# JuanTarrio/rebvo

Measured on AMD Instinct MI355X. Metric: frames/sec (DoG+extract+track+depth) 752x480 EuRoC, higher is better.
Workload: dtype f32 scale-space / f64 tracker+EKF

## Files before the change

### include/edgehip.h

```cpp
#ifndef EDGEHIP_H
#define EDGEHIP_H
#include <stdint.h>

#ifdef __cplusplus
extern "C" {
#endif

#define EDGEHIP_ABI_VERSION 2
#define EDGEHIP_KEYLINE_MAX 50000

typedef enum edgehip_status {
    EDGEHIP_OK = 0,
    EDGEHIP_ERR_ARG = -1,
    EDGEHIP_ERR_DEVICE = -2,
    EDGEHIP_ERR_MEMORY = -3,
    EDGEHIP_ERR_STATE = -4
} edgehip_status;

typedef struct edgehip_ctx edgehip_ctx;

typedef struct edgehip_params {
    int32_t w, h;
    double ppx, ppy, zfx, zfy;
    double kc[5];
// ... 28 lines not shown
    int32_t p_id, n_id, net_id, stereo_m_id;
    double stereo_rho, stereo_s_rho;
} edgehip_keyline;

typedef struct edgehip_seq_state {
    double tresh;
    double V[3], W[3];
    double P_V[9], P_W[9];
    double R[9];
    double Pose[9], Pos[3];
    double Kp, P_Kp, K;
    double s_rho_q;
    double score, rel_error, rel_error_score;
    double t_prev, dt;
    float retuned_thresh;
    int32_t l_kl_num;
    int32_t frame;
    int32_t klm_fwd;
    int32_t klm_num, kf_matchs;
    int32_t estimation_ok;
    int32_t minimizer_evals;
} edgehip_seq_state;

typedef struct edgehip_nav {
    double t, dt;
    double V[3], W[3], P_V[9], P_W[9];
    double Rot[9], RotLie[3], Vel[3], Pose[9], PoseLie[3], Pos[3];
    double Kp, RKp, s_rho_q, tresh, score, rel_error, rel_error_score;
    float retuned_thresh;
    int32_t kn, klm_fwd, klm_num, kf_matchs, estimation_ok, frame, minimizer_evals;
} edgehip_nav;

typedef struct edgehip_imu_params {
    double giro_meas_std, giro_bias_std;
    int32_t init_bias, init_bias_frame_num;
    double bias_init_guess[3];
    double acel_meas_std, g_module, g_module_uncer, g_uncert, vbias_std;
    double scale_std_mult, scale_std_max, scale_std_init;
} edgehip_imu_params;
typedef struct edgehip_imu_integrated {
    int32_t n, pad;
    double dt, Rot[9], giro[3], acel[3], comp[3], dgiro[3], cacel[3];
} edgehip_imu_integrated;
typedef struct edgehip_nav_imu {
    double Rot[9], RotLie[3], RotGiro[3], Vel[3], Pose[9], PoseLie[3], Pos[3], g[3];
    double scale, dt, K, Kp, RKp, s_rho_q;
    double Vg[3], Bg[3], dVv[3], dWv[3], Vgv[3], Vgva[3], Av[3], As[3], X[7], b_est[3], u_est[3];
    int32_t kn, klm_num, estimation_ok, init;
} edgehip_nav_imu;

int edgehip_create(const edgehip_params *params, int nseq, int nslots, int device, edgehip_ctx **out);
int edgehip_destroy(edgehip_ctx *ctx);
const char *edgehip_last_error(void);
int edgehip_abi_version(void);
int edgehip_experiments(void);
int edgehip_sync(edgehip_ctx *ctx);
void *edgehip_stream(edgehip_ctx *ctx);
int edgehip_box_widths(edgehip_ctx *ctx, int out[6]);

int edgehip_upload_rgb(edgehip_ctx *ctx, int slot, const uint8_t *rgb24, int seq_first, int count);
int edgehip_upload_rgb_device(edgehip_ctx *ctx, int slot, const void *rgb24_dev);
int edgehip_alloc_pinned(size_t bytes, void **out);
int edgehip_free_pinned(void *p);
int edgehip_upload_rgb_pinned(edgehip_ctx *ctx, int slot, const uint8_t *rgb24_pinned, int seq_first, int count);
int edgehip_upload_sync(edgehip_ctx *ctx);
int edgehip_upload_wait(edgehip_ctx *ctx, int slot);

int edgehip_upload_rgb_indexed(edgehip_ctx *ctx, int slot, const void *pool_dev, int pool_frames, const int32_t *idx);
int edgehip_bind_rgb_indexed(edgehip_ctx *ctx, int slot, const void *pool_dev, int pool_frames, const int32_t *idx);
int edgehip_upload_grey8(edgehip_ctx *ctx, int slot, const uint8_t *grey8, int seq_first, int count);
int edgehip_upload_grey8_pinned(edgehip_ctx *ctx, int slot, const uint8_t *grey8_pinned, int seq_first, int count);
int edgehip_bind_grey8_indexed(edgehip_ctx *ctx, int slot, const void *pool_dev, int pool_frames, const int32_t *idx);

int edgehip_stage_a(edgehip_ctx *ctx, int slot);
int edgehip_get_kn(edgehip_ctx *ctx, int slot, int32_t *kn_out);

int edgehip_quantile(edgehip_ctx *ctx, int slot, double s_rho_min, double s_rho_max, double pct, int nbins);
int edgehip_build_field(edgehip_ctx *ctx, int slot, int radius, float min_mod);
int edgehip_try_velrot(edgehip_ctx *ctx, int slot_new, int slot_old, const double *X, int reweight, int procjf,
                       double match_thresh, const double *s_rho_min, uint32_t match_num_thresh, double k_huber,
                       int resid_in, int resid_out, double *out);
int edgehip_download_resid(edgehip_ctx *ctx, int which, double *resid);
int edgehip_minimizer_rv(edgehip_ctx *ctx, int slot_new, int slot_old);
int edgehip_set_tracker_precision(edgehip_ctx *ctx, int bits);
int edgehip_lm_solve(edgehip_ctx *ctx, const double *A, const double *b, int n, int svd_rule, double *h);

typedef struct edgehip_kf_request {
    double X0[6];
    double Kr;
    double max_s_rho;
} edgehip_kf_request;
typedef struct edgehip_kf_result {
    double X[6];
    double RRV[36];
    double score_ratio;
    double F, F0;
    int32_t evals, mnum;
} edgehip_kf_result;
int edgehip_minimizer_rv_kf(edgehip_ctx *ctx, int slot_kf, int slot_cur, const edgehip_kf_request *req, double match_mod,
                            double match_ang, double rho_tol, int iter_max, double reweight_distance, uint32_t match_num_thresh,
                            edgehip_kf_result *res);

int edgehip_minimizer_v(edgehip_ctx *ctx, int slot_new, int slot_old, double *V, const double *s_rho_min, float min_mod,
                        double match_thresh, int iter_max, uint32_t match_num_thresh, double reweight_distance,
                        double *RVel, double *F);

int edgehip_forward_match(edgehip_ctx *ctx, int slot_old, int slot_new);
int edgehip_rotate_keylines(edgehip_ctx *ctx, int slot, const double *R );
int edgehip_directed_matching(edgehip_ctx *ctx, int slot_new, int slot_old);
int edgehip_match_one_pass(edgehip_ctx *ctx, int slot_new, int slot_old, int fill);
int edgehip_regularize_ekf(edgehip_ctx *ctx, int slot, int do_regularize, int do_ekf);
int edgehip_ext_rot_vel(edgehip_ctx *ctx, int slot, const double *vel, double loc_unc, double hub_reweight, double *X,
                        double *Wx, double *Rx, int32_t *ok);
int edgehip_rescale(edgehip_ctx *ctx, int slot);

int edgehip_set_slot_camera(edgehip_ctx *ctx, int slot, double ppx, double ppy, double zfx, double zfy);
int edgehip_directed_matching_stereo(edgehip_ctx *ctx, int slot, int slot_pair, const double *t, const double *R,
                                     double min_thr_mod, double min_thr_ang, double max_radius, double loc_unc,
                                     double q_abs, double q_rel, double loc_unc_model, int32_t *nmatch);
int edgehip_fuse_stereo_depth(edgehip_ctx *ctx, int slot);
int edgehip_set_stereo_rig(edgehip_ctx *ctx, int slot_pair, const double *t, const double *R, double max_radius);
int edgehip_get_stereo_matches(edgehip_ctx *ctx, int32_t *nmatch);

int edgehip_process_frame(edgehip_ctx *ctx, const double *t);
int edgehip_next_slot(edgehip_ctx *ctx);
int edgehip_cur_slot(edgehip_ctx *ctx);
int edgehip_read_nav(edgehip_ctx *ctx, edgehip_nav *nav);
int edgehip_imu_enable(edgehip_ctx *ctx, const edgehip_imu_params *imu);
int edgehip_set_imu(edgehip_ctx *ctx, const edgehip_imu_integrated *per_seq);
int edgehip_read_nav_imu(edgehip_ctx *ctx, edgehip_nav_imu *out);
int edgehip_set_nav_log(edgehip_ctx *ctx, int len);
int edgehip_read_nav_log(edgehip_ctx *ctx, int first, int count, edgehip_nav *out);
int edgehip_read_nav_log_device(edgehip_ctx *ctx, int first, int count, void *out_dev);
int edgehip_read_nav_imu_log(edgehip_ctx *ctx, int first, int count, edgehip_nav_imu *out);
int edgehip_read_stereo_matches_log(edgehip_ctx *ctx, int first, int count, int32_t *out);
int edgehip_reset(edgehip_ctx *ctx);
int edgehip_depth_reset(edgehip_ctx *ctx, int seq);
int edgehip_depth_reset_slot(edgehip_ctx *ctx, int seq, int slot);

int edgehip_get_state(edgehip_ctx *ctx, int seq, edgehip_seq_state *out);
int edgehip_set_state(edgehip_ctx *ctx, int seq, const edgehip_seq_state *in);
int edgehip_get_framecount(edgehip_ctx *ctx, int seq, int slot, uint32_t *fc);
int edgehip_set_framecount(edgehip_ctx *ctx, int seq, int slot, uint32_t fc);
int edgehip_download_keylines(edgehip_ctx *ctx, int seq, int slot, edgehip_keyline *kl, int32_t *mask,
                              int32_t *kn_out);
int edgehip_download_keylines_batch(edgehip_ctx *ctx, int slot, int n, const int32_t *seqs, edgehip_keyline *const *kl, int32_t *kn_out);
int edgehip_export_keylines(edgehip_ctx *ctx, int n, const int32_t *seqs, int *ticket_out);
int edgehip_export_fetch(edgehip_ctx *ctx, int ticket, const int32_t *kn, edgehip_keyline *const *dst);
int edgehip_export_wait(edgehip_ctx *ctx, int ticket);
int edgehip_register_host(void *p, size_t bytes);
int edgehip_unregister_host(void *p);
int edgehip_upload_keylines(edgehip_ctx *ctx, int seq, int slot, const edgehip_keyline *kl, int32_t kn,
                            const int32_t *mask, float retuned_thresh);
int edgehip_download_plane(edgehip_ctx *ctx, int seq, int which, float *out);
int edgehip_download_field(edgehip_ctx *ctx, int seq, int32_t *out);
int edgehip_build_undistort_map(const edgehip_params *params, int32_t *inx, int32_t *iw);
int edgehip_download_undistorted(edgehip_ctx *ctx, int seq, int slot, uint8_t *rgb24);

typedef enum edgehip_bound_mode {
    EDGEHIP_BOUND_NONE = 0,
    EDGEHIP_BOUND_CORNERS = 1,
    EDGEHIP_BOUND_FULL = 2
} edgehip_bound_mode;
typedef struct edgehip_depth_fill_params {
    int32_t block_w, block_h;
    int32_t iter_num;
// ... 192 lines not shown
```

### rebvo_amd/csrc/api.hip

```cpp

#include <math.h>
#include <stdio.h>
#include <stdlib.h>
#include <string.h>

#include <algorithm>
#include <mutex>

#include "ctx.h"
#include "stage_a_dev.h"

namespace edgehip {

static thread_local std::string g_err;

int wait_pinned_ring(edgehip_ctx *c) {
    const int r = c->frames_seen % 8;
    if (c->ring_valid[r]) EH_CHECK(hipEventSynchronize(c->ev_ring[r]));
    return 0;
}

static int wait_idx_row(edgehip_ctx *c, int slot, const int32_t *pi) {
    if (c->slot_src[slot].idx_row != pi) return 0;
    if (c->a_api_valid[slot]) EH_CHECK(hipEventSynchronize(c->ev_a[slot]));
// ... 354 lines not shown
        EH_CHECK(hipEventCreateWithFlags(&c->ev_a[i], hipEventDisableTiming));
        EH_CHECK(hipEventCreateWithFlags(&c->ev_use[i], hipEventDisableTiming));
        c->use_valid[i] = false;
    }
    EH_CHECK(hipEventCreateWithFlags(&c->ev_tmp, hipEventDisableTiming));
    EH_CHECK(hipEventCreateWithFlags(&c->ev_stage, hipEventDisableTiming));
    EH_CHECK(hipEventCreateWithFlags(&c->ev_stage8, hipEventDisableTiming));
    for (int i = 0; i < 8; i++) { EH_CHECK(hipEventCreateWithFlags(&c->ev_ring[i], hipEventDisableTiming)); c->ring_valid[i] = false; }
    if (nslots > 4) { set_error("edgehip_create: at most 4 frame slots"); return EDGEHIP_ERR_ARG; }

    DevicePlan &pl = c->plan;
    pl.w = p.w; pl.h = p.h; pl.n = p.w * p.h; pl.nseq = nseq; pl.nslots = nslots;
    pl.ftx = (p.w + 3) / 4;
    pl.fstride = (size_t)pl.ftx * (size_t)((p.h + 3) / 4) * 16;
    pl.f16tx = (p.w + 7) / 8;
    pl.f16stride = (size_t)pl.f16tx * (size_t)((p.h + 3) / 4) * 32;
    pl.cap = std::min(p.max_points, EDGEHIP_KEYLINE_MAX);
    const double sr0 = kovesi_boxes(p.sigma0, kMaxBoxes, pl.box[0]);
    kovesi_boxes(sr0 * p.ksigma, kMaxBoxes, pl.box[1]);
    for (int f = 0; f < 2; f++)
        for (int i = 0; i < kMaxBoxes; i++) {
            if (pl.box[f][i] < 1 || pl.box[f][i] * pl.box[f][i] >= kDivLutMax) {
                set_error("edgehip_create: box width out of range for these sigmas");
                return EDGEHIP_ERR_ARG;
            }
            pl.box_a[f][i] = (float)(1.0 / (pl.box[f][i] * pl.box[f][i]));
        }
    pl.ppx = (float)p.ppx; pl.ppy = (float)p.ppy; pl.zfx = (float)p.zfx; pl.zfy = (float)p.zfy;
    pl.zfm = (double)((pl.zfx + pl.zfy) / 2);

    const size_t B = nseq, S = nslots, N = pl.n, CAP = pl.cap;
    int e;
#define EH_TRY(x) if ((e = (x)) != 0) return e
    EH_TRY(dmalloc(c, &c->rgb, S * B * N * 3 + 16, al->dev, 0));
    EH_TRY(dmalloc(c, &c->ii, 4 * B * N, al->dev, 0));
    c->planes = nullptr;
    if (p.debug_planes) EH_TRY(dmalloc(c, &c->planes, 5 * B * N, al->dev, 0));
    EH_TRY(dmalloc(c, &c->mask, S * B * N, al->dev, 0xFF));
    EH_TRY(dmalloc(c, &c->field, B * pl.fstride, al->dev, 0xFF));
    EH_TRY(dmalloc(c, &c->field16, B * pl.f16stride, al->dev, 0));
    c->field32_valid = false;
    c->und_base = nullptr;
    c->und_iw = nullptr;
    if (p.use_undistort) {
        EH_TRY(dmalloc(c, &c->und_base, N, al->dev));
        EH_TRY(dmalloc(c, &c->und_iw, N, al->dev));
        std::vector<int32_t> base;
        std::vector<uint32_t> iw;
        build_undistort_map(p, base, iw, nullptr, nullptr);
        EH_CHECK(hipMemcpy(c->und_base, base.data(), sizeof(int32_t) * N, hipMemcpyHostToDevice));
        EH_CHECK(hipMemcpy(c->und_iw, iw.data(), sizeof(uint32_t) * 4 * N, hipMemcpyHostToDevice));
    }
    EH_TRY(dmalloc(c, &c->div_lut, kDivLutMax, al->dev));
    EH_TRY(dmalloc(c, &c->pinv, 3 * 49, al->dev, 0));
    EH_TRY(dmalloc(c, &c->seq, B, al->dev, 0));
    EH_TRY(dmalloc(c, &c->seqa, B, al->dev, 0));
    EH_TRY(dmalloc(c, &c->tresh_slot, S * B, al->dev, 0));
    c->fc_rows = std::max<int>(nslots, kRefRing);
    c->fc_index = 0;
    EH_TRY(dmalloc(c, &c->framecount, (size_t)c->fc_rows * B, al->dev, 0));
    EH_TRY(dmalloc(c, &c->kn_slot, S * B, al->dev, 0));
    EH_TRY(dmalloc(c, &c->retuned_slot, S * B, al->dev, 0));
    c->band_rows = detect_band_rows(p.w, p.plane_fit_size);
    c->nbands = (p.h - 2 * p.plane_fit_size + c->band_rows - 1) / c->band_rows;
    {
        const int npx = c->band_rows * p.w, nchunk = (npx + 63) / 64, cpw = (nchunk + kDetWaves - 1) / kDetWaves;
        c->band_cap = cpw * 64;
    }
    const size_t nstrips = (size_t)c->nbands * kDetWaves;
    EH_TRY(dmalloc(c, &c->band_cnt, B * nstrips, al->dev, 0));
    EH_TRY(dmalloc(c, &c->band_off, B * (nstrips + 1), al->dev, 0));
    {
        char *bs;
        EH_TRY(dmalloc(c, &bs, B * nstrips * c->band_cap * 20, al->dev));
        c->band_stage = bs;
    }
    EH_TRY(dmalloc(c, &c->histo, B * 256, al->dev, 0));
    c->nblk_tvr = (int)((CAP + kTvrBlock - 1) / kTvrBlock);
    EH_TRY(dmalloc(c, &c->P0, B * 3 * CAP, al->dev, 0));
    EH_TRY(dmalloc(c, &c->resid, (size_t)kResidBufs * B * CAP, al->dev, 0));
    EH_TRY(dmalloc(c, &c->resid_carry, (size_t)kResidBufs * B * c->nblk_tvr, al->dev, 0));
    EH_TRY(dmalloc(c, &c->partials, 2 * B * c->nblk_tvr * kNumSums, al->dev, 0));
    EH_TRY(dmalloc(c, &c->block_last, 2 * B * c->nblk_tvr, al->dev, 0));
    EH_TRY(dmalloc(c, &c->bin_cnt, B * 256, al->dev, 0));
    {
        const size_t ntiles = (size_t)((p.w + 63) / 64) * ((p.h + 63) / 64);
        EH_TRY(dmalloc(c, &c->bins, B * ntiles * CAP, al->dev));
    }
    c->field_radius = p.search_range;
    c->field_mode = EH_EXP_ENV("EDGEHIP_FIELD_MODE", 0);
    c->no_grec = getenv("EDGEHIP_NO_GREC") && atoi(getenv("EDGEHIP_NO_GREC")) != 0;
    c->level_mode = getenv("EDGEHIP_LEVEL_MODE") ? atoi(getenv("EDGEHIP_LEVEL_MODE")) : 0;
    c->fwd_mode = EH_EXP_ENV("EDGEHIP_FWD_MODE", 0);
    c->fused_min_batch = fused_min_env;
    c->fused_undist = EH_EXP_ENV("EDGEHIP_FUSED_UNDIST", 0) != 0;
    c->tvr_rw2 = EH_EXP_ENV("EDGEHIP_TVR_RW2", 0);
    c->dual_init = getenv("EDGEHIP_DUAL_INIT") ? atoi(getenv("EDGEHIP_DUAL_INIT")) : 1;
    c->persist_lm_max = EH_EXP_ENV("EDGEHIP_PERSIST_LM", 0);
    EH_TRY(dmalloc(c, &c->sync_cnt, B, al->dev, 0));
    EH_TRY(dmalloc(c, &c->fwd_key, B * CAP, al->dev, 0));
    EH_TRY(dmalloc(c, &c->fwd_win, B * CAP, al->dev, 0xFF));
    EH_TRY(dmalloc(c, &c->rs_tmp, B * 2 * CAP, al->dev, 0));
    c->fuse_match = !(getenv("EDGEHIP_FUSE_MATCH") && atoi(getenv("EDGEHIP_FUSE_MATCH")) == 0);
    if (c->fuse_match) {
        EH_TRY(dmalloc(c, &c->rot_pm, S * B * CAP, al->dev, 0)); EH_TRY(dmalloc(c, &c->rot_mm, S * B * CAP, al->dev, 0));
        EH_TRY(dmalloc(c, &c->rot_rho, S * B * CAP, al->dev, 0)); EH_TRY(dmalloc(c, &c->rot_srho, S * B * CAP, al->dev, 0));
    }
    EH_TRY(dmalloc(c, &c->rot_buf, B * 9, al->dev, 0));
    EH_TRY(dmalloc(c, &c->nav_dev, B, al->dev, 0));
    EH_TRY(dmalloc(c, &c->idx_dev, B, al->dev, 0));
    c->slot_src.assign(S, edgehip_ctx::SlotSrc());
    c->stereo_cnt = nullptr;
    if (p.stereo_available) EH_TRY(dmalloc(c, &c->stereo_cnt, B, al->dev, 0));
    c->nav_log = nullptr;
    c->nav_log_len = 0;

    {
        const size_t al256 = 256;
        auto up = [&](size_t x) { return (x + al256 - 1) / al256 * al256; };
        const bool stereo = p.stereo_available != 0;
        const size_t per = up(CAP * 4) * 8  +
                           up(CAP * 8) * 6  + up(CAP * 8) * 7  + up(CAP * 32) + up(CAP * 16)  +
                           (stereo ? up(CAP * 4) + 2 * up(CAP * 8) : 0);
        char *arena;
        EH_TRY(dmalloc(c, &arena, per * S * B, al->dev, 0));
        c->kl_arena = arena;
        c->kl.resize(S * B);
        for (size_t sb = 0; sb < S * B; sb++) {
            char *q = arena + sb * per;
            KlSoA &k = c->kl[sb];
            auto take = [&](size_t bytes) { char *r = q; q += up(bytes); return r; };
            k.p_inx = (int32_t *)take(CAP * 4);
            k.m_m = (float2 *)take(CAP * 8); k.u_m = (float2 *)take(CAP * 8); k.c_p = (float2 *)take(CAP * 8);
            k.p_m = (float2 *)take(CAP * 8); k.p_m_0 = (float2 *)take(CAP * 8); k.m_m0 = (float2 *)take(CAP * 8);
            k.n_m = (float *)take(CAP * 4);
            k.rho = (double *)take(CAP * 8); k.s_rho = (double *)take(CAP * 8); k.rho_nr = (double *)take(CAP * 8);
            k.s_rho_nr = (double *)take(CAP * 8); k.rho0 = (double *)take(CAP * 8); k.s_rho0 = (double *)take(CAP * 8);
            k.n_m0 = (double *)take(CAP * 8);
            k.m_id = (int32_t *)take(CAP * 4); k.m_id_f = (int32_t *)take(CAP * 4); k.m_id_kf = (int32_t *)take(CAP * 4);
            k.m_num = (int32_t *)take(CAP * 4); k.p_id = (int32_t *)take(CAP * 4); k.n_id = (int32_t *)take(CAP * 4);
            k.rec = (MatchRec *)take(CAP * 32);
            k.grec = (float4 *)take(CAP * 16);
            k.stereo_m_id = nullptr; k.stereo_rho = nullptr; k.stereo_s_rho = nullptr;
            if (stereo) {
                k.stereo_m_id = (int32_t *)take(CAP * 4);
                k.stereo_rho = (double *)take(CAP * 8); k.stereo_s_rho = (double *)take(CAP * 8);
            }
        }
        c->slot_cam.assign(S, edgehip_ctx::SlotCam{pl.ppx, pl.ppy, pl.zfm});
        EH_TRY(dmalloc(c, &c->kl_dev, S * B, al->dev));
        EH_CHECK(hipMemcpyAsync(c->kl_dev, c->kl.data(), sizeof(KlSoA) * S * B, hipMemcpyHostToDevice, c->stream));
    }
    {
        std::vector<float> lut(kDivLutMax, 0.f);
        for (int k = 1; k < kDivLutMax; k++) lut[k] = (float)(1.0 / (double)(float)k);
        EH_CHECK(hipMemcpyAsync(c->div_lut, lut.data(), sizeof(float) * kDivLutMax, hipMemcpyHostToDevice, c->stream));
        double pinv[3 * 49] = {0};
        plane_fit_pinv(p.plane_fit_size, pinv);
        if (p.plane_fit_size == 2)
            for (int i = 0; i < 5; i++)
                for (int j = 0; j < 5; j++) {
                    const int k = i * 5 + j;
                    if (!(pinv[k] == pinv[j] && pinv[25 + k] == pinv[25 + 5 * i] && pinv[50 + k] == pinv[50])) {
                        set_error("edgehip_create: plane-fit pseudo inverse lost its separable structure");
                        return EDGEHIP_ERR_STATE;
                    }
// ... 999 lines not shown
```

### rebvo_amd/csrc/ctx.h

```cpp
#pragma once
#include <hip/hip_runtime.h>
#include <stdint.h>
#include <string.h>
#include <string>
#include <map>
#include <vector>
#include <mutex>
#include <atomic>

#include "edgehip.h"
#include "export_ring.h"

namespace edgehip {

constexpr int kMaxBoxes = 3;
constexpr int kBandRows = 12;
constexpr int kDetWaves = 16;
constexpr int kDivLutMax = 256;
constexpr int kTvrThreads = 256;
constexpr int kTvrBlock = kTvrThreads;
constexpr int kNumSums = 28;
constexpr int kRefRing = 8;
constexpr int kResidBufs = 3;

// ... 266 lines not shown
    typedef T __attribute__((address_space(1))) G;
    __builtin_nontemporal_store(v, (G *)p + i);
#else
    st_stream(p + i, v);
#endif
}
__device__ __forceinline__ void stg_stream(float2 *p, size_t i, float2 v) {
#if EDGEHIP_GLOBAL_LD
    typedef float f2v __attribute__((ext_vector_type(2)));
    typedef f2v __attribute__((address_space(1))) G;
    __builtin_nontemporal_store(f2v{v.x, v.y}, (G *)p + i);
#else
    st_stream(p + i, v);
#endif
}
#endif

struct Profiler;

}

struct edgehip_ctx {
    edgehip_params p;
    edgehip::DevicePlan plan;
    int device;
    hipStream_t stream;
    hipStream_t stream_a;
    hipEvent_t ev_a[4];
    hipEvent_t ev_use[4];
    hipEvent_t ev_tmp;
    hipEvent_t ev_stage, ev_stage8;
    bool stage_busy = false, stage8_busy = false;
    hipStream_t stream_up;
    hipEvent_t ev_up[4];
    bool up_valid[4];
    int slot_ring[4];
    bool no_grec;
    bool grec_ok[4];
    bool rec_stale[4];
    bool rig_a_valid = false;
    bool capturing = false;
    bool a_api_valid[4];
    hipEvent_t ev_ring[8];
    bool ring_valid[8];
    bool use_valid[4];
    int overlap;
    bool lds_optin_level = false, lds_optin_detect = false, lds_optin_fused = false;
    bool lds_optin_rescale = false;
    int frame_slot;
    int frames_seen;
    uint8_t *rgb;
    float *ii;
    float *planes;
    int32_t *mask;
    uint32_t *field;
    uint16_t *field16;
    bool field32_valid;
    int32_t *und_base;
    uint4 *und_iw;
    float *div_lut;
    double *pinv;
    void *kl_arena;
    std::vector<edgehip::KlSoA> kl;
    edgehip::KlSoA *kl_dev;
    edgehip::SeqDev *seq;
    edgehip::SeqA *seqa;
    double *tresh_slot;
    uint32_t *framecount;
    int fc_rows;
    int fc_index;
    int32_t *kn_slot;
    float *retuned_slot;
    int32_t *band_cnt;
    int32_t *band_off;
    void *band_stage;
    int nbands, band_cap;
    int band_rows;
    int32_t *histo;
    double *P0;
    double *resid;
    double *resid_carry;
    double *partials;
    double *block_last;
    bool use_graph;
    std::map<int, hipGraphExec_t> frame_graphs;
    struct StereoRig {
        bool enabled = false;
        int slot_pair = -1;
        double t[3], R[9], max_radius;
    } rig;
    int ring_slots;
    struct SlotSrc { const uint8_t *base = nullptr; std::vector<int32_t> host_idx; bool grey8 = false;
                     const int32_t *idx_row = nullptr; int idx_ring = 0; };
    uint8_t *grey8 = nullptr;
    uint8_t *pinned_grey8 = nullptr;
    std::vector<SlotSrc> slot_src;
    struct SlotCam { float ppx, ppy; double zfm; };
    std::vector<SlotCam> slot_cam;
    int field_radius;
    int field_mode;
    int level_mode;
    int fused_min_batch;
    double pinv_host[3 * 49];
    int32_t *bin_cnt;
    int32_t *bins;
    int nblk_tvr;
    bool fused_undist;
    int tvr_rw2;
    bool tracker_f32 = false;
    int dual_init;
    int persist_lm_max;
    unsigned *sync_cnt;
    unsigned long long *fwd_key;
    int32_t *fwd_win;
    int fwd_mode = 0;
    bool fuse_match = true;
    float2 *rot_pm = nullptr, *rot_mm = nullptr;
    double *rot_rho = nullptr, *rot_srho = nullptr;
    bool rot_pending[4] = {false, false, false, false};
    bool fwd_fill[4] = {false, false, false, false};
    bool fwd_cleared = false;
    bool fwd_keys_posted = false;
    bool fwd_key_in_tvr = false;
    double *rs_tmp;
    double *rot_buf;
    const double *t_src = nullptr;
    edgehip_keyline *aos_dev = nullptr;
    edgehip_keyline *aos_host = nullptr;
    int32_t *aos_req_dev = nullptr, *aos_req_host = nullptr;
    int aos_requests = 0;
    edgehip::ExportRing kl_ring;
    edgehip::ExportRing ros_ring;
    edgehip_nav *nav_dev;
    edgehip_nav *nav_log;
    edgehip_nav_imu *nav_imu_log = nullptr;
    int nav_log_len;
    int32_t *stereo_log = nullptr;
    hipStream_t stream_log = nullptr;
    hipEvent_t ev_log = nullptr;
    hipEvent_t ev_log_ring[8] = {};
    std::mutex log_mu;
    std::atomic<long long> frames_logged{0};
    long long log_first = 0, log_last = -1;
    int32_t *idx_dev;
    int32_t *stereo_cnt;
    uint8_t *pinned_rgb;
    size_t pinned_rgb_bytes;
    edgehip::SeqDev *pinned_seq;
    edgehip::SeqA *pinned_seqa;
    double *pinned_out;
    double *pinned_t;
    int32_t *pinned_idx;
    edgehip_nav *pinned_nav;
    edgehip::Profiler *prof;
    bool imu_enabled = false, imu_pending = false;
    bool imu_pinned_ok = false;
    edgehip_imu_params imu_params;
    edgehip_kf_request *kf_req_dev = nullptr;
    edgehip_kf_result *kf_res_dev = nullptr;
    void *imu_track = nullptr;
    void *imu_filter = nullptr;
    void *imu_snap = nullptr;
    hipStream_t stream_imu = nullptr;
    hipEvent_t ev_imu_snap[2], ev_imu_post[2];
    hipEvent_t ev_imu_mid[2];
    bool imu_post_valid[2] = {false, false};
// ... 168 lines not shown
```

### rebvo_amd/csrc/stage_b.hip

```cpp

#include <math.h>
#include <string.h>

#include <vector>

#include <type_traits>

#include "ctx.h"
#include "resid_carry.h"
#include "wave_reduce.h"

namespace edgehip {

struct RetuneArgs {
    SeqA *seqa;
    const int32_t *histo;
    float *retuned_out;
    int knum, nbins;
};
template <int NT>
__global__ __launch_bounds__(NT) void k_quantile(const KlSoA *kls, const int32_t *__restrict__ kns, SeqDev *seqs,
                                                 double smin, double smax, double pct, int nbins, const double *__restrict__ t_in, double fps,
                                                 RetuneArgs rt) {
    __shared__ int s_h[256];
// ... 403 lines not shown
                acc_abl += val | off;
#else
                atomicMin(px, val);
#endif
            };
            constexpr int UNROLL = EDGEHIP_RASTER_UNROLL;
            const float t1f = (float)t1;
            float tf = (float)t0;
            if constexpr (UNROLL > 1) {
                for (; tf + (float)(UNROLL - 1) <= t1f; tf += (float)UNROLL) {
#pragma unroll
                    for (int j = 0; j < UNROLL; j++) sample(tf + (float)j);
                }
            }
            for (; tf <= t1f; tf += 1.f) sample(tf);
#if EDGEHIP_RASTER_ABL == 2
            if (acc_abl == 0x12345u) s_tile[1] = acc_abl;
#endif
        }
    };
    using T = std::true_type;
    using F = std::false_type;
    if (tx0 == 0) { if (ty0 == 0) raster(T{}, T{}); else raster(T{}, F{}); }
    else { if (ty0 == 0) raster(F{}, T{}); else raster(F{}, F{}); }
    __syncthreads();
    if (tid == 0) bin_cnt[(size_t)seq * kMaxTiles + tile] = 0;
#if EDGEHIP_RASTER_ABL == 4
    if (s_tile[tid] != 0x12345u) return;
#endif
    if (keep32) {
        uint32_t *out = field + (size_t)seq * fstride;
        for (int i = tid; i < FT * FT; i += 256) {
            const int st = i >> 4, in = i & 15;
            const int lx = ((st % (FT / 4)) << 2) | (in & 3), ly = ((st / (FT / 4)) << 2) | (in >> 2);
            const int x = tx0 + lx, y = ty0 + ly;
            if (x < w && y < h) out[field_index(x, y, ftx)] = s_tile[ly * TS + lx];
        }
    }
    uint16_t *o16 = field16 + (size_t)seq * f16stride;
    for (int i = tid; i < FT * FT / 2; i += 256) {
        const int st = i >> 4, in = i & 15;
        const int lx = ((st % (FT / 8)) << 3) | ((in & 3) << 1), ly = ((st / (FT / 8)) << 2) | (in >> 2);
        const int x = tx0 + lx, y = ty0 + ly;
        if (x < w && y < h) {
            const uint32_t v0 = s_tile[ly * TS + lx], v1 = s_tile[ly * TS + lx + 1];
            const uint32_t a0 = v0 == 0xFFFFFFFFu ? 0u : ((0x10000u - (v0 & 0xFFFFu)) & 0xFFFFu);
            const uint32_t a1 = v1 == 0xFFFFFFFFu ? 0u : ((0x10000u - (v1 & 0xFFFFu)) & 0xFFFFu);
#if EDGEHIP_NT_RASTER
            st_stream(reinterpret_cast<uint32_t *>(o16 + field16_index(x, y, f16tx)), a0 | (a1 << 16));
#else
            *reinterpret_cast<uint32_t *>(o16 + field16_index(x, y, f16tx)) = a0 | (a1 << 16);
#endif
        }
    }
}

__global__ __launch_bounds__(256) void k_field_to16(const uint32_t *__restrict__ field, uint16_t *__restrict__ f16, int w, int h,
                                                    size_t fstride, int ftx, size_t f16stride, int f16tx) {
    const int seq = blockIdx.z;
    const size_t e = (size_t)blockIdx.x * 256 + threadIdx.x;
    if (e >= f16stride) return;
    const size_t tile = e >> 5; const int in = (int)(e & 31);
    const int x = (int)(tile % (size_t)f16tx) * 8 + (in & 7), y = (int)(tile / (size_t)f16tx) * 4 + (in >> 3);
    uint16_t v = 0;
    if (x < w && y < h) {
        const uint32_t f = field[(size_t)seq * fstride + field_index(x, y, ftx)];
        if (f != 0xFFFFFFFFu) v = (uint16_t)(0xFFFF - (int)(f & 0xFFFFu) + 1);
    }
    f16[(size_t)seq * f16stride + e] = v;
}

__global__ __launch_bounds__(256) void k_tvr_prepare(const KlSoA *kls, const int32_t *__restrict__ kns, double *__restrict__ P0,
                                                     double *__restrict__ resid0, double *__restrict__ carry0, SeqDev *seqs,
                                                     int cap, int nblk, double zfm) {
    const int seq = blockIdx.z;
    const int i = blockIdx.x * 256 + threadIdx.x;
    const int kn = kns[seq];
    if (i == 0) seqs[seq].kn_old = kn;
    if ((i % kTvrBlock) == 0 && i / kTvrBlock < nblk) carry0[(size_t)seq * nblk + i / kTvrBlock] = 0.0;
    if (i >= kn) return;
    resid0[(size_t)seq * cap + i] = 0.0;
}

__device__ __forceinline__ void so3_exp_inl(const double (&w)[3], double (&R)[9]) {
    const double one_6th = 1.0 / 6.0, one_20th = 1.0 / 20.0;
    const double theta_sq = w[0] * w[0] + w[1] * w[1] + w[2] * w[2];
    const double theta = sqrt(theta_sq);
    double A, B;
    if (theta_sq < 1e-8) {
        A = 1.0 - one_6th * theta_sq;
        B = 0.5;
    } else if (theta_sq < 1e-6) {
        B = 0.5 - 0.25 * one_6th * theta_sq;
        A = 1.0 - theta_sq * one_6th * (1.0 - one_20th * theta_sq);
    } else {
        const double inv_theta = 1.0 / theta;
        A = sin(theta) * inv_theta;
        B = (1 - cos(theta)) * (inv_theta * inv_theta);
    }
    const double wx2 = w[0] * w[0], wy2 = w[1] * w[1], wz2 = w[2] * w[2];
    R[0] = 1.0 - B * (wy2 + wz2);
    R[4] = 1.0 - B * (wx2 + wz2);
    R[8] = 1.0 - B * (wx2 + wy2);
    double a = A * w[2], b = B * (w[0] * w[1]);
    R[1] = b - a; R[3] = b + a;
    a = A * w[1]; b = B * (w[0] * w[2]);
    R[2] = b + a; R[6] = b - a;
    a = A * w[0]; b = B * (w[1] * w[2]);
    R[5] = b - a; R[7] = b + a;
}
__device__ __noinline__ void so3_exp(const double w[3], double R[9]) {
    const double wv[3] = {w[0], w[1], w[2]};
    double Rr[9];
    so3_exp_inl(wv, Rr);
    for (int i = 0; i < 9; i++) R[i] = Rr[i];
}

__device__ __noinline__ void tvr_setup(SeqDev *sq, const double *X) {
    double R0[9], Rz[9];
    so3_exp(X + 3, R0);
    const double wz[3] = {0.0, 0.0, X[5]};
    so3_exp(wz, Rz);
    for (int i = 0; i < 9; i++) sq->Rt[i] = R0[i];
    sq->RM[0] = Rz[0]; sq->RM[1] = Rz[1]; sq->RM[2] = Rz[3]; sq->RM[3] = Rz[4];
    for (int i = 0; i < 3; i++) sq->Vt[i] = X[i];
}


__device__ __forceinline__ void tvr_setup2(SeqDev *sq, const double *X, const int lane, const bool zero = false, const int l0 = 0) {
    if (lane >= l0 && lane < l0 + 2) {
        const bool first = lane == l0;
        const double wv[3] = {first ? X[3] : 0.0, first ? X[4] : 0.0, X[5]};
        double R[9];
        so3_exp_inl(wv, R);
        double *Rt = zero ? sq->zRt : sq->Rt, *Vt = zero ? sq->zVt : sq->Vt, *RM = zero ? sq->zRM : sq->RM;
        if (first) {
            for (int i = 0; i < 9; i++) Rt[i] = R[i];
            for (int i = 0; i < 3; i++) Vt[i] = X[i];
        } else {
            RM[0] = R[0]; RM[1] = R[1]; RM[2] = R[3]; RM[3] = R[4];
        }
    }
}


struct TvrArgs {
    const KlSoA *kl_old;
    const KlSoA *kl_new;
    const int32_t *kn_old;
    const uint16_t *field16;
    const double *P0;
    double *resid;
    double *resid_carry;
    double *block_last;
    double *partials;
    double *block_last_z;
    double *partials_z;
    SeqDev *seq;
    const uint32_t *framecount;
    int w, h, cap, nblk, nseq;
    size_t f16stride;
    int f16tx;
    double zfm, max_r, match_thresh, k_huber, inv_k_huber;
    double inv_zfm;
    float ppx, ppy;
    uint32_t match_num_thresh;
    int write_mid;
    int use_grec;
    unsigned long long *fwd_key;
    const edgehip_kf_request *kf;
    double kf_match_mod, kf_match_cang, kf_rho_tol;
};

__device__ __forceinline__ double rsqrt_f64(double x) {
    double y = __builtin_amdgcn_rsq(x);
    const double hx = 0.5 * x;
    y = y * (1.5 - hx * y * y);
    y = y * (1.5 - hx * y * y);
    return x > 1e300 ? 0.0 : y;
}

#ifndef EDGEHIP_TVR_MFMA
#define EDGEHIP_TVR_MFMA 0
#endif
#ifndef EDGEHIP_TVR_REF_ORDER
#define EDGEHIP_TVR_REF_ORDER 1
#endif
#ifndef EDGEHIP_TVR_ABL
#define EDGEHIP_TVR_ABL 0
#endif
template <bool GREC>
__device__ __forceinline__ void load_matched(const KlSoA &kl, const int ikf, float &cpx, float &cpy, float &mx, float &my, float &ux, float &uy) {
    if (GREC) {
        const float4 g = ldg(kl.grec, ikf);
        cpx = g.x; cpy = g.y; mx = g.z; my = g.w;
    } else {
        const MatchRec fr = kl.rec[ikf];
        cpx = fr.c_px; cpy = fr.c_py; mx = fr.m_mx; my = fr.m_my; ux = fr.u_mx; uy = fr.u_my;
    }
}
__device__ __forceinline__ void grec_u_m(const float mx, const float my, float &ux, float &uy) {
    const float n2m = mx * mx + my * my;
    const float nm = sqrtf_mid(n2m);
    div2_mid_f32(mx, my, nm, ux, uy);
}

template <typename T>
__device__ __forceinline__ void jac_row(T (&J)[6], const T zf, const T rho_p, const T pix, const T piy, const T ptx, const T pty, const T ptz,
                                        const T dfx, const T dfy) {
    T t0 = zf * rho_p;
    J[0] = t0 * dfx;
    J[1] = t0 * dfy;
    t0 = rho_p * pix;
    J[2] = t0 * dfx;
    t0 = rho_p * piy;
    J[2] += t0 * dfy;
    J[3] = J[1] * ptz; J[3] += J[2] * pty;
    J[4] = J[0] * ptz; J[4] += J[2] * ptx;
    t0 = J[0] * pty;
    J[5] = (T)-1 * t0; J[5] += J[1] * ptx;
}

template <bool REWEIGHT, bool PROCJF, bool GREC, bool KF = false>
__device__ __forceinline__ void tvr_body(const TvrArgs &a, const int seq, const int blk, const int tid) {
    constexpr int ABL = KF ? 0 : EDGEHIP_TVR_ABL;
    const int lane = tid & 63, wave = tid >> 6;
    SeqDev *sq = a.seq + seq;
    const int kn = a.kn_old[seq];
    if (blk * kTvrBlock >= kn) return;
    const KlSoA &ko = a.kl_old[seq];
    const int res_in = sq->res_cur, res_out = sq->lm_phase == 0 ? sq->res_t : sq->res_new;
    const double *rin = a.resid + ((size_t)res_in * a.nseq + seq) * a.cap;
    double *rout = a.resid + ((size_t)res_out * a.nseq + seq) * a.cap;
    const double carry_in_prev = a.resid_carry[((size_t)res_in * a.nseq + seq) * a.nblk + blk];

    constexpr int NW = kTvrThreads / 64;
    constexpr bool GRAM_MFMA = PROCJF && EDGEHIP_TVR_MFMA && !(ABL & 1);
    __shared__ double s_rows[GRAM_MFMA ? NW : 1][GRAM_MFMA ? 64 : 1][8];
    __shared__ double s_wlast[NW];
    __shared__ int s_whas[NW];
    double sums[kNumSums];
#pragma unroll
    for (int i = 0; i < kNumSums; i++) sums[i] = 0;

    const int ikl = blk * kTvrBlock + tid;
    double J[6] = {0, 0, 0, 0, 0, 0};
    double fm, dfx, dfy;
    double ptx, pty, ptz, pix, piy, rho_p, s_rho;
#if EDGEHIP_TVR_REF_ORDER
    double wgt_ref;
#else
    double inv_w2 = 1;
#endif
    int mid_f = -1;
    int status = 0;
    double fi = 0;
    double rho_own;
    if (ikl < kn) {
        s_rho = ldg(ko.s_rho, ikl);
        const int32_t mnum = ldg(ko.m_num, ikl);
        const float2 pm0 = ldg(ko.p_m, ikl);
        const double rho0 = ldg(ko.rho, ikl);
        rho_own = rho0;
        const float2 klm = ldg(ko.m_m, ikl);
        const float knm = ldg(ko.n_m, ikl);
        double rprev = 0;
        if (REWEIGHT && !(ABL & 16)) rprev = rin[ikl];
        const uint32_t fc = KF ? 0xFFFFFFFFu : a.framecount[seq];
        const uint32_t mthr = a.match_num_thresh < fc ? a.match_num_thresh : fc;
        const bool skip = s_rho > sq->s_rho_min_eval || (uint32_t)mnum < mthr;
        if (!skip) {
            const double sz = inv_mid(rho0);
            const double pz_zf0 = a.inv_zfm * sz;
            const double sx = pz_zf0 * (double)pm0.x, sy = pz_zf0 * (double)pm0.y;
            const double *R = sq->Rt, *V = sq->Vt;
            ptx = R[0] * sx; ptx += R[1] * sy; ptx += R[2] * sz; ptx = V[0] + ptx;
            pty = R[3] * sx; pty += R[4] * sy; pty += R[5] * sz; pty = V[1] + pty;
            ptz = R[6] * sx; ptz += R[7] * sy; ptz += R[8] * sz; ptz = V[2] + ptz;
            rho_p = inv_mid(ptz);
            const double pz_zf = a.zfm * rho_p;
            pix = pz_zf * ptx;
            piy = pz_zf * pty;
            const double px = pix + (double)a.ppx, py = piy + (double)a.ppy;
            const int x = cvt_trunc_sat_i32(px + 0.5), y = cvt_trunc_sat_i32(py + 0.5);
            dfx = 0; dfy = 0;
#if EDGEHIP_TVR_REF_ORDER
            wgt_ref = 1;
#endif
            if (REWEIGHT) {
                if (is_carry(rprev)) rprev = carry_in_prev;
#if EDGEHIP_TVR_REF_ORDER
                if (fabs(rprev) > a.k_huber) wgt_ref = div_mid(a.k_huber, fabs(rprev));
#else
                if (fabs(rprev) > a.k_huber && !(ABL & 2)) { const double rk = fabs(rprev) * a.inv_k_huber; inv_w2 = rk * rk; }
#endif
            }
            fm = a.max_r;
            if (x < 1 || y < 1 || x >= a.w - 1 || y >= a.h - 1) {
                status = 1;
            } else {
                status = 3;
                const float rmx = KF ? klm.x : (float)(sq->RM[0] * (double)klm.x + sq->RM[1] * (double)klm.y);
                const float rmy = KF ? klm.y : (float)(sq->RM[2] * (double)klm.x + sq->RM[3] * (double)klm.y);
                const uint32_t f = (ABL & 8) ? (uint32_t)(ikl + 1) : a.field16[(size_t)seq * a.f16stride + field16_index(x, y, a.f16tx)];
                if (KF) {
                    if (f != 0u) {
                        const int ikf = (int)f - 1;
                        const KlSoA &kf = a.kl_new[seq];
                        const MatchRec fr = kf.rec[ikf];
                        const double f_rho = kf.rho[ikf], f_srho = kf.s_rho[ikf];
                        const double cang = (double)((klm.x * fr.m_mx + klm.y * fr.m_my) / knm);
                        const double rho_t = rho_p / a.kf[seq].Kr;
                        const bool reject = cang < a.kf_match_cang || (double)fabsf(knm / fr.n_m - 1) > a.kf_match_mod ||
                                            fabs(rho_t - f_rho) > a.kf_rho_tol * (f_srho + s_rho * rho_t / rho0);
                        if (!reject) {
                            const double dx = px - (double)fr.c_px, dy = py - (double)fr.c_py;
                            fi = dx * (double)fr.u_mx + dy * (double)fr.u_my;
                            dfx = (double)fr.u_mx;
                            dfy = (double)fr.u_my;
                            fm = fi;
                            mid_f = ikf;
                            status = 2;
                        }
                    }
                } else {
                    const int ikf = f != 0u ? (int)f - 1 : 0;
                    float f_cpx, f_cpy, f_mx, f_my, f_ux, f_uy;
                    if (ABL & 4) {
                        f_cpx = (float)px; f_cpy = (float)py; f_mx = klm.x; f_my = klm.y; f_ux = 1.f; f_uy = 0.f;
                    } else {
                        load_matched<GREC>(a.kl_new[seq], ikf, f_cpx, f_cpy, f_mx, f_my, f_ux, f_uy);
                    }
                    const double p_n2 = (double)(knm * knm);
                    const double p_esc = (double)(rmx * f_mx + rmy * f_my);
                    if ((f != 0u) & !(fabs(p_esc - p_n2) > a.match_thresh * p_n2)) {
                        if (GREC) grec_u_m(f_mx, f_my, f_ux, f_uy);
                        const double dx = px - (double)f_cpx, dy = py - (double)f_cpy;
                        fi = dx * (double)f_ux + dy * (double)f_uy;
                        dfx = (double)f_ux;
                        dfy = (double)f_uy;
                        fm = fi;
                        mid_f = ikf;
                        status = 2;
                    }
                }
            }
        }
    }

    {
        const WaveLast<double> wl = wave_last_valid(fi, status == 2, lane);
        carry_publish(wl, lane, wave, s_wlast, s_whas);
        __syncthreads();
        if (status == 3) {
            rout[ikl] = carry_inherit(wl, wave, s_wlast, s_whas);
        } else if (status == 2) {
            rout[ikl] = fi;
        } else if (status == 1) {
            rout[ikl] = a.max_r;
        } else if (ikl < kn) {
            rout[ikl] = 0.0;
        }
    }
    if (a.write_mid && ikl < kn) {
        stg(ko.m_id_f, ikl, mid_f);
        if (!KF && a.fwd_key && mid_f >= 0) atomicMax(&a.fwd_key[(size_t)seq * a.cap + mid_f], ord_bits(rho_own));
    }

    double fs = 0;
    if (status != 0) {
#if EDGEHIP_TVR_REF_ORDER
        if (REWEIGHT) { fm *= wgt_ref; dfx *= wgt_ref; dfy *= wgt_ref; }
#endif
        if (PROCJF) jac_row(J, a.zfm, rho_p, pix, piy, ptx, pty, ptz, dfx, dfy);
        const double qvel = (a.zfm * dfx * sq->Vt[0] + a.zfm * dfy * sq->Vt[1] + (pix * dfx + piy * dfy) * sq->Vt[2]);
#if EDGEHIP_TVR_REF_ORDER
        const double q_rho = REWEIGHT ? sqrt_ge1(s_rho * qvel * s_rho * qvel + 1) : s_rho;
        const double r_q = rcp_for_div_rn(q_rho);
        if (PROCJF) {
#pragma unroll
            for (int j = 0; j < 6; j++) J[j] = div_rn(J[j], q_rho, r_q);
        }
        fs = div_rn(fm, q_rho, r_q);
#else
        double inv_q;
        if (REWEIGHT) {
            const double sq = s_rho * qvel;
            inv_q = (ABL & 2) ? sq + inv_w2 : rsqrt_f64(sq * sq + inv_w2);
        } else {
            inv_q = 1.0 / s_rho;
        }
        if (PROCJF) {
#pragma unroll
            for (int j = 0; j < 6; j++) J[j] *= inv_q;
        }
        fs = fm * inv_q;
#endif
    } else if (!REWEIGHT && !KF && ikl < kn && s_rho == 0) {
        const double qnan = __longlong_as_double(0x7ff8000000000000ll);
        if (PROCJF) {
#pragma unroll
            for (int j = 0; j < 6; j++) J[j] = qnan;
        }
        fs = qnan;
    }
    if (GRAM_MFMA) {
        double2 *row = reinterpret_cast<double2 *>(&s_rows[wave][lane][0]);
        row[0] = make_double2(J[0], J[1]);
        row[1] = make_double2(J[2], J[3]);
        row[2] = make_double2(J[4], J[5]);
        row[3] = make_double2(fs, 0.0);
    } else {
        int ns = 0;
        if (PROCJF) {
#pragma unroll
            for (int i = 0; i < 6; i++)
#pragma unroll
                for (int j = i; j < 6; j++) sums[ns++] = J[i] * J[j];
#pragma unroll
            for (int i = 0; i < 6; i++) sums[ns++] = J[i] * fs;
        }
        sums[PROCJF ? ns : kNumSums - 1] = fs * fs;
    }

    if (tid == 0) a.block_last[(size_t)seq * a.nblk + blk] = carry_block_last(s_wlast, s_whas);

    __shared__ double s_red[NW][32];
    if (GRAM_MFMA) {
        typedef double v4d __attribute__((ext_vector_type(4)));
        __builtin_amdgcn_fence(__ATOMIC_RELEASE, "wavefront");
        __builtin_amdgcn_wave_barrier();
        const int m = (lane & 15) < 7 ? (lane & 15) : 7, kk = lane >> 4;
        const double *src = &s_rows[wave][kk][m];
        v4d acc = {0.0, 0.0, 0.0, 0.0};
#pragma unroll
        for (int st = 0; st < 16; st++) {
            const double v = src[st * 4 * 8];
            acc = __builtin_amdgcn_mfma_f64_16x16x4f64(v, v, acc, 0, 0, 0);
        }
        const int j = lane & 15;
#pragma unroll
        for (int r = 0; r < 2; r++) {
            const int i = (lane >> 4) + 4 * r;
            if (j < 7 && i <= j) {
                const int idx = j < 6 ? i * 6 - (i * (i - 1)) / 2 + (j - i) : (i < 6 ? 21 + i : 27);
                s_red[wave][idx] = acc[r];
            }
        }
    } else if (PROCJF && (ABL & 1)) {
        if (lane < kNumSums) s_red[wave][lane] = sums[lane % 4];
    } else {
        block_reduce_put<PROCJF>(sums, lane, wave, s_red);
    }
    __syncthreads();
    block_reduce_store<PROCJF>(s_red, tid, a.partials + ((size_t)seq * a.nblk + blk) * kNumSums);
}

template <bool REWEIGHT, bool PROCJF, bool GREC>
__global__ __launch_bounds__(kTvrThreads) void k_try_velrot(TvrArgs a) {
    tvr_body<REWEIGHT, PROCJF, GREC>(a, blockIdx.z, blockIdx.x, threadIdx.x);
}
__global__ __launch_bounds__(kTvrThreads) void k_try_velrot_kf(TvrArgs a) {
    tvr_body<true, true, false, true>(a, blockIdx.z, blockIdx.x, threadIdx.x);
}

template <bool REWEIGHT, bool PROCJF, bool GREC>
__device__ __forceinline__ void tvr_body_f32(const TvrArgs &a, const int seq, const int blk, const int tid) {
    const int lane = tid & 63, wave = tid >> 6;
    SeqDev *sq = a.seq + seq;
    const int kn = a.kn_old[seq];
    if (blk * kTvrBlock >= kn) return;
    const KlSoA &ko = a.kl_old[seq];
    const int res_in = sq->res_cur, res_out = sq->lm_phase == 0 ? sq->res_t : sq->res_new;
    const double *rin = a.resid + ((size_t)res_in * a.nseq + seq) * a.cap;
    double *rout = a.resid + ((size_t)res_out * a.nseq + seq) * a.cap;
    const double carry_in_prev = a.resid_carry[((size_t)res_in * a.nseq + seq) * a.nblk + blk];
    constexpr int NW = kTvrThreads / 64;
    __shared__ float s_wlast[NW];
    __shared__ int s_whas[NW];
    float sums[kNumSums];
#pragma unroll
    for (int i = 0; i < kNumSums; i++) sums[i] = 0.f;

    const int ikl = blk * kTvrBlock + tid;
    float J[6] = {0, 0, 0, 0, 0, 0};
    float fm, dfx, dfy;
    float ptx, pty, ptz, pix, piy, rho_p;
    double s_rho;
    float wgt;
    int mid_f = -1, status = 0;
    float fi = 0;
    double rho_own;
    const float zf = (float)a.zfm, max_r = (float)a.max_r, k_huber = (float)a.k_huber, simil_t = (float)a.match_thresh;
    float Vt0, Vt1, Vt2;
    if (ikl < kn) {
        s_rho = ldg(ko.s_rho, ikl);
        const int32_t mnum = ldg(ko.m_num, ikl);
        const float2 pm0 = ldg(ko.p_m, ikl);
        const double rho0 = ldg(ko.rho, ikl);
        rho_own = rho0;
        const float2 klm = ldg(ko.m_m, ikl);
        const float knm = ldg(ko.n_m, ikl);
        double rprev_d = 0;
        if (REWEIGHT) rprev_d = rin[ikl];
        const uint32_t fc = a.framecount[seq];
        const uint32_t mthr = a.match_num_thresh < fc ? a.match_num_thresh : fc;
        const bool skip = s_rho > sq->s_rho_min_eval || (uint32_t)mnum < mthr;
        Vt0 = (float)sq->Vt[0]; Vt1 = (float)sq->Vt[1]; Vt2 = (float)sq->Vt[2];
        if (!skip) {
            const float sz = 1.f / (float)rho0;
            const float pz_zf0 = (1.f / zf) * sz;
            const float sx = pz_zf0 * pm0.x, sy = pz_zf0 * pm0.y;
            const double *Rd = sq->Rt;
            const float R0 = (float)Rd[0], R1 = (float)Rd[1], R2 = (float)Rd[2], R3 = (float)Rd[3], R4 = (float)Rd[4], R5 = (float)Rd[5],
                        R6 = (float)Rd[6], R7 = (float)Rd[7], R8 = (float)Rd[8];
            ptx = R0 * sx; ptx += R1 * sy; ptx += R2 * sz; ptx = Vt0 + ptx;
            pty = R3 * sx; pty += R4 * sy; pty += R5 * sz; pty = Vt1 + pty;
            ptz = R6 * sx; ptz += R7 * sy; ptz += R8 * sz; ptz = Vt2 + ptz;
            rho_p = 1.f / ptz;
            const float pz_zf = zf * rho_p;
            pix = pz_zf * ptx;
            piy = pz_zf * pty;
            const float px = pix + a.ppx, py = piy + a.ppy;
            const int x = cvt_trunc_sat_i32((double)px + 0.5), y = cvt_trunc_sat_i32((double)py + 0.5);
            dfx = 0; dfy = 0; wgt = 1;
            if (REWEIGHT) {
                if (is_carry(rprev_d)) rprev_d = carry_in_prev;
                const float rprev = (float)rprev_d;
                if (fabsf(rprev) > k_huber) wgt = k_huber / fabsf(rprev);
            }
            fm = max_r;
            if (x < 1 || y < 1 || x >= a.w - 1 || y >= a.h - 1) {
                status = 1;
            } else {
                status = 3;
                const float rmx = (float)sq->RM[0] * klm.x + (float)sq->RM[1] * klm.y;
                const float rmy = (float)sq->RM[2] * klm.x + (float)sq->RM[3] * klm.y;
                const uint32_t f = a.field16[(size_t)seq * a.f16stride + field16_index(x, y, a.f16tx)];
                {
                    const int ikf = f != 0u ? (int)f - 1 : 0;
                    float f_cpx, f_cpy, f_mx, f_my, f_ux, f_uy;
                    load_matched<GREC>(a.kl_new[seq], ikf, f_cpx, f_cpy, f_mx, f_my, f_ux, f_uy);
                    const float p_n2 = knm * knm;
                    const float p_esc = rmx * f_mx + rmy * f_my;
                    if ((f != 0u) & !(fabsf(p_esc - p_n2) > simil_t * p_n2)) {
                        if (GREC) grec_u_m(f_mx, f_my, f_ux, f_uy);
                        const float dx = px - f_cpx, dy = py - f_cpy;
                        fi = dx * f_ux + dy * f_uy;
                        dfx = f_ux;
                        dfy = f_uy;
                        fm = fi;
                        mid_f = ikf;
                        status = 2;
                    }
                }
            }
        }
    }
    {
        const WaveLast<float> wl = wave_last_valid(fi, status == 2, lane);
        carry_publish(wl, lane, wave, s_wlast, s_whas);
        __syncthreads();
        if (status == 3) {
            rout[ikl] = carry_inherit(wl, wave, s_wlast, s_whas);
        } else if (status == 2) {
            rout[ikl] = (double)fi;
        } else if (status == 1) {
            rout[ikl] = (double)max_r;
        } else if (ikl < kn) {
            rout[ikl] = 0.0;
        }
    }
    if (a.write_mid && ikl < kn) {
        stg(ko.m_id_f, ikl, mid_f);
        if (a.fwd_key && mid_f >= 0) atomicMax(&a.fwd_key[(size_t)seq * a.cap + mid_f], ord_bits(rho_own));
    }
    float fs = 0.f;
    if (status != 0) {
        if (REWEIGHT) { fm *= wgt; dfx *= wgt; dfy *= wgt; }
        if (PROCJF) jac_row(J, zf, rho_p, pix, piy, ptx, pty, ptz, dfx, dfy);
        const double qvel = (double)(zf * dfx * Vt0 + zf * dfy * Vt1 + (pix * dfx + piy * dfy) * Vt2);
        const double q_rho = REWEIGHT ? sqrt_ge1(s_rho * qvel * s_rho * qvel + 1) : s_rho;
        const double r_q = rcp_for_div_rn(q_rho);
        if (PROCJF) {
#pragma unroll
            for (int j = 0; j < 6; j++) J[j] = (float)div_rn((double)J[j], q_rho, r_q);
        }
        fs = (float)div_rn((double)fm, q_rho, r_q);
    }
    {
        int ns = 0;
        if (PROCJF) {
#pragma unroll
            for (int i = 0; i < 6; i++)
#pragma unroll
                for (int j = i; j < 6; j++) sums[ns++] = J[i] * J[j];
#pragma unroll
            for (int i = 0; i < 6; i++) sums[ns++] = J[i] * fs;
        }
        sums[PROCJF ? ns : kNumSums - 1] = fs * fs;
    }
    if (tid == 0) a.block_last[(size_t)seq * a.nblk + blk] = carry_block_last(s_wlast, s_whas);
    __shared__ float s_red[NW][32];
    block_reduce_put<PROCJF>(sums, lane, wave, s_red);
    __syncthreads();
    block_reduce_store<PROCJF>(s_red, tid, a.partials + ((size_t)seq * a.nblk + blk) * kNumSums);
}
template <bool REWEIGHT, bool PROCJF, bool GREC>
__global__ __launch_bounds__(kTvrThreads) void k_try_velrot_f32(TvrArgs a) {
    tvr_body_f32<REWEIGHT, PROCJF, GREC>(a, blockIdx.z, blockIdx.x, threadIdx.x);
}

#ifndef EDGEHIP_TVR2_PARK
#define EDGEHIP_TVR2_PARK 1
#endif
template <bool PROCJF, bool GREC>
__device__ __forceinline__ void tvr2_body(const TvrArgs &a, const int seq, const int blk, const int tid) {
    const int lane = tid & 63, wave = tid >> 6;
    SeqDev *sq = a.seq + seq;
    const int kn = a.kn_old[seq];
    if (blk * kTvrBlock >= kn) return;
    const KlSoA &ko = a.kl_old[seq];
    double *rout0 = a.resid + ((size_t)sq->res_t * a.nseq + seq) * a.cap;
    double *rout1 = a.resid + ((size_t)sq->res_new * a.nseq + seq) * a.cap;
    constexpr int NW = kTvrThreads / 64;
    __shared__ double s_wlast[2][NW];
    __shared__ int s_whas[2][NW];

    const int ikl = blk * kTvrBlock + tid;
    double fm[2], dfx[2], dfy[2], fi[2] = {0, 0};
    double ptx[2], pty[2], ptz[2], pix[2], piy[2], rho_p[2];
    int status[2] = {0, 0};
    double s_rho = 1;
    if (ikl < kn) {
        s_rho = ldg(ko.s_rho, ikl);
        const int32_t mnum = ldg(ko.m_num, ikl);
        const float2 pm0 = ldg(ko.p_m, ikl);
        const double rho0 = ldg(ko.rho, ikl);
        const float2 klm = ldg(ko.m_m, ikl);
        const float knm = ldg(ko.n_m, ikl);
        const uint32_t fc = a.framecount[seq];
        const uint32_t mthr = a.match_num_thresh < fc ? a.match_num_thresh : fc;
        const bool skip = s_rho > sq->s_rho_min_eval || (uint32_t)mnum < mthr;
        if (!skip) {
            const double sz = inv_mid(rho0);
            const double pz_zf0 = a.inv_zfm * sz;
            const double sx = pz_zf0 * (double)pm0.x, sy = pz_zf0 * (double)pm0.y;
            double px[2], py[2];
            bool inimg[2];
            size_t fidx[2];
            float rmx[2], rmy[2];
#pragma unroll
            for (int c = 0; c < 2; c++) {
                const double *R = c ? sq->Rt : sq->zRt, *V = c ? sq->Vt : sq->zVt, *RM = c ? sq->RM : sq->zRM;
                ptx[c] = R[0] * sx; ptx[c] += R[1] * sy; ptx[c] += R[2] * sz; ptx[c] = V[0] + ptx[c];
                pty[c] = R[3] * sx; pty[c] += R[4] * sy; pty[c] += R[5] * sz; pty[c] = V[1] + pty[c];
                ptz[c] = R[6] * sx; ptz[c] += R[7] * sy; ptz[c] += R[8] * sz; ptz[c] = V[2] + ptz[c];
                rho_p[c] = inv_mid(ptz[c]);
                const double pz_zf = a.zfm * rho_p[c];
                pix[c] = pz_zf * ptx[c];
                piy[c] = pz_zf * pty[c];
                px[c] = pix[c] + (double)a.ppx; py[c] = piy[c] + (double)a.ppy;
                const int x = x86_cvttsd2si(px[c] + 0.5), y = x86_cvttsd2si(py[c] + 0.5);
                inimg[c] = !(x < 1 || y < 1 || x >= a.w - 1 || y >= a.h - 1);
                fidx[c] = inimg[c] ? field16_index(x, y, a.f16tx) : (size_t)0;
                rmx[c] = (float)(RM[0] * (double)klm.x + RM[1] * (double)klm.y);
                rmy[c] = (float)(RM[2] * (double)klm.x + RM[3] * (double)klm.y);
                fm[c] = a.max_r;
                dfx[c] = 0; dfy[c] = 0;
                status[c] = inimg[c] ? 3 : 1;
            }
            const uint16_t *fld = a.field16 + (size_t)seq * a.f16stride;
            const uint32_t f0 = fld[fidx[0]], f1 = fld[fidx[1]];
            const bool hit0 = inimg[0] && f0 != 0u, hit1 = inimg[1] && f1 != 0u;
            const int ikf0 = hit0 ? (int)f0 - 1 : 0, ikf1 = hit1 ? (int)f1 - 1 : 0;
            float f_cpx[2], f_cpy[2], f_mx[2], f_my[2], f_ux[2] = {0, 0}, f_uy[2] = {0, 0};
            load_matched<GREC>(a.kl_new[seq], ikf0, f_cpx[0], f_cpy[0], f_mx[0], f_my[0], f_ux[0], f_uy[0]);
            load_matched<GREC>(a.kl_new[seq], ikf1, f_cpx[1], f_cpy[1], f_mx[1], f_my[1], f_ux[1], f_uy[1]);
            const double p_n2 = (double)(knm * knm);
#pragma unroll
            for (int c = 0; c < 2; c++) {
                {
                    const double p_esc = (double)(rmx[c] * f_mx[c] + rmy[c] * f_my[c]);
                    if ((c ? hit1 : hit0) & !(fabs(p_esc - p_n2) > a.match_thresh * p_n2)) {
                        if (GREC) grec_u_m(f_mx[c], f_my[c], f_ux[c], f_uy[c]);
                        const double dx = px[c] - (double)f_cpx[c], dy = py[c] - (double)f_cpy[c];
                        fi[c] = dx * (double)f_ux[c] + dy * (double)f_uy[c];
                        dfx[c] = (double)f_ux[c];
                        dfy[c] = (double)f_uy[c];
                        fm[c] = fi[c];
                        status[c] = 2;
                    }
                }
            }
        }
    }

    WaveLast<double> wl[2];
#pragma unroll
    for (int c = 0; c < 2; c++) {
        wl[c] = wave_last_valid(fi[c], status[c] == 2, lane);
        carry_publish(wl[c], lane, wave, s_wlast[c], s_whas[c]);
    }
    __syncthreads();
#pragma unroll
    for (int c = 0; c < 2; c++) {
        double *rout = c ? rout1 : rout0;
        if (status[c] == 3) {
            rout[ikl] = carry_inherit(wl[c], wave, s_wlast[c], s_whas[c]);
        } else if (status[c] == 2) {
            rout[ikl] = fi[c];
        } else if (status[c] == 1) {
            rout[ikl] = a.max_r;
        } else if (ikl < kn) {
            rout[ikl] = 0.0;
        }
    }
    if (tid == 0) {
#pragma unroll
        for (int c = 0; c < 2; c++)
            (c ? a.block_last : a.block_last_z)[(size_t)seq * a.nblk + blk] = carry_block_last(s_wlast[c], s_whas[c]);
    }

    __shared__ double s_red[2][NW][32];
#if EDGEHIP_TVR2_PARK
    __shared__ double s_park[PROCJF ? 7 : 1][kTvrThreads];
#endif
    const double inv_q = rcp_for_div_rn(s_rho);
    double Jc[2][6], fmc[2];
#pragma unroll
    for (int c = 0; c < 2; c++) {
        double (&J)[6] = Jc[c];
#pragma unroll
        for (int j = 0; j < 6; j++) J[j] = 0;
        fmc[c] = 0;
        if (status[c] != 0) {
            fmc[c] = fm[c];
            if (PROCJF) {
                jac_row(J, a.zfm, rho_p[c], pix[c], piy[c], ptx[c], pty[c], ptz[c], dfx[c], dfy[c]);
#if EDGEHIP_TVR_REF_ORDER
#pragma unroll
                for (int j = 0; j < 6; j++) J[j] = div_rn(J[j], s_rho, inv_q);
#else
#pragma unroll
                for (int j = 0; j < 6; j++) J[j] *= inv_q;
#endif
            }
#if EDGEHIP_TVR_REF_ORDER
            fmc[c] = div_rn(fmc[c], s_rho, inv_q);
#else
            fmc[c] *= inv_q;
#endif
        } else if (ikl < kn && s_rho == 0) {
            const double qnan = __longlong_as_double(0x7ff8000000000000ll);
            if (PROCJF) {
#pragma unroll
                for (int j = 0; j < 6; j++) J[j] = qnan;
            }
            fmc[c] = qnan;
        }
    }
#if EDGEHIP_TVR2_PARK
    if (PROCJF) {
#pragma unroll
        for (int j = 0; j < 6; j++) s_park[j][tid] = Jc[1][j];
        s_park[6][tid] = fmc[1];
    }
#endif
#pragma unroll
    for (int c = 0; c < 2; c++) {
        if (PROCJF) {
            double J[6], f;
#if EDGEHIP_TVR2_PARK
            if (c == 1) {
#pragma unroll
                for (int j = 0; j < 6; j++) J[j] = s_park[j][tid];
                f = s_park[6][tid];
            } else
#endif
            {
#pragma unroll
                for (int j = 0; j < 6; j++) J[j] = Jc[c][j];
                f = fmc[c];
            }
            double sums[kNumSums];
            int ns = 0;
#pragma unroll
            for (int i = 0; i < 6; i++)
#pragma unroll
                for (int j = i; j < 6; j++) sums[ns++] = J[i] * J[j];
#pragma unroll
            for (int i = 0; i < 6; i++) sums[ns++] = J[i] * f;
            sums[ns] = f * f;
            block_reduce_put<true>(sums, lane, wave, s_red[c]);
        } else {
            block_reduce_put_score(fmc[c] * fmc[c], lane, wave, s_red[c]);
        }
    }
    __syncthreads();
    if (wave < 2) {
        const int c = 1 - wave;
        block_reduce_store<PROCJF>(s_red[c], lane, (c ? a.partials : a.partials_z) + ((size_t)seq * a.nblk + blk) * kNumSums);
    }
}

template <bool PROCJF, bool GREC>
__device__ __forceinline__ void tvr2_body_f32(const TvrArgs &a, const int seq, const int blk, const int tid) {
    const int lane = tid & 63, wave = tid >> 6;
    SeqDev *sq = a.seq + seq;
    const int kn = a.kn_old[seq];
    if (blk * kTvrBlock >= kn) return;
    const KlSoA &ko = a.kl_old[seq];
    double *rout0 = a.resid + ((size_t)sq->res_t * a.nseq + seq) * a.cap;
    double *rout1 = a.resid + ((size_t)sq->res_new * a.nseq + seq) * a.cap;
    constexpr int NW = kTvrThreads / 64;
    __shared__ float s_wlast[2][NW];
    __shared__ int s_whas[2][NW];
    const float zf = (float)a.zfm, max_r = (float)a.max_r, simil_t = (float)a.match_thresh;

    const int ikl = blk * kTvrBlock + tid;
    float fm[2] = {0, 0}, dfx[2] = {0, 0}, dfy[2] = {0, 0}, fi[2] = {0, 0};
    float ptx[2] = {0, 0}, pty[2] = {0, 0}, ptz[2] = {1, 1}, pix[2] = {0, 0}, piy[2] = {0, 0}, rho_p[2] = {1, 1};
    int status[2] = {0, 0};
    double s_rho = 1;
    if (ikl < kn) {
        s_rho = ldg(ko.s_rho, ikl);
        const int32_t mnum = ldg(ko.m_num, ikl);
        const float2 pm0 = ldg(ko.p_m, ikl);
        const double rho0 = ldg(ko.rho, ikl);
        const float2 klm = ldg(ko.m_m, ikl);
        const float knm = ldg(ko.n_m, ikl);
        const uint32_t fc = a.framecount[seq];
        const uint32_t mthr = a.match_num_thresh < fc ? a.match_num_thresh : fc;
        const bool skip = s_rho > sq->s_rho_min_eval || (uint32_t)mnum < mthr;
        if (!skip) {
            const float sz = 1.f / (float)rho0;
// ... 225 lines not shown
    }
    WaveLast<double> wl[2];
#pragma unroll
    for (int c = 0; c < 2; c++) {
        wl[c] = wave_last_valid(fi[c], status[c] == 2, lane);
        carry_publish(wl[c], lane, wave, s_wlast[c], s_whas[c]);
    }
    __syncthreads();
#pragma unroll
    for (int c = 0; c < 2; c++) {
        if (status[c] == 3) {
            rout[ikl[c]] = carry_inherit(wl[c], wave, s_wlast[c], s_whas[c]);
        } else if (status[c] == 2) {
            rout[ikl[c]] = fi[c];
        } else if (status[c] == 1) {
            rout[ikl[c]] = a.max_r;
        } else if (ikl[c] < kn) {
            rout[ikl[c]] = 0.0;
        }
        if (a.write_mid && ikl[c] < kn) {
            ko.m_id_f[ikl[c]] = mid_f[c];
            if (a.fwd_key && mid_f[c] >= 0) atomicMax(&a.fwd_key[(size_t)seq * a.cap + mid_f[c]], ord_bits(rho_own[c]));
        }
    }
    if (tid == 0) {
#pragma unroll
        for (int c = 0; c < 2; c++) {
            if ((2 * blk + c) * kTvrBlock >= kn || 2 * blk + c >= a.nblk) continue;
            a.block_last[(size_t)seq * a.nblk + 2 * blk + c] = carry_block_last(s_wlast[c], s_whas[c]);
        }
    }
    double sums[kNumSums];
#pragma unroll
    for (int i = 0; i < kNumSums; i++) sums[i] = 0;
#pragma unroll
    for (int c = 0; c < 2; c++) {
        double J[6] = {0, 0, 0, 0, 0, 0};
        double fmc = fm[c];
        if (ikl[c] < kn) {
#if EDGEHIP_TVR_REF_ORDER
            fmc *= inv_w2[c]; dfx[c] *= inv_w2[c]; dfy[c] *= inv_w2[c];
#endif
            jac_row(J, a.zfm, rho_p[c], pix[c], piy[c], ptx[c], pty[c], ptz[c], dfx[c], dfy[c]);
            const double qvel = (a.zfm * dfx[c] * V[0] + a.zfm * dfy[c] * V[1] + (pix[c] * dfx[c] + piy[c] * dfy[c]) * V[2]);
#if EDGEHIP_TVR_REF_ORDER
            const double q_rho = sqrt(s_rho[c] * qvel * s_rho[c] * qvel + 1), r_q = 1.0 / q_rho;
#pragma unroll
            for (int j = 0; j < 6; j++) J[j] = div_rn(J[j], q_rho, r_q);
            fmc = div_rn(fmc, q_rho, r_q);
#else
            const double sq_ = s_rho[c] * qvel;
            const double inv_q = rsqrt_f64(sq_ * sq_ + inv_w2[c]);
#pragma unroll
            for (int j = 0; j < 6; j++) J[j] *= inv_q;
            fmc *= inv_q;
#endif
        }
        int ns = 0;
#pragma unroll
        for (int i = 0; i < 6; i++)
#pragma unroll
            for (int j = i; j < 6; j++) sums[ns++] += J[i] * J[j];
#pragma unroll
        for (int i = 0; i < 6; i++) sums[ns++] += J[i] * fmc;
        sums[ns] += fmc * fmc;
    }
    __shared__ double s_red[NW][32];
    double *prow = a.partials + ((size_t)seq * a.nblk + 2 * blk) * kNumSums;
    block_reduce_put<true>(sums, lane, wave, s_red);
    __syncthreads();
    block_reduce_store<true>(s_red, tid, prow);
    if (tid < kNumSums && 2 * blk + 1 < a.nblk) prow[kNumSums + tid] = 0.0;
}

template <bool GREC>
__global__ __launch_bounds__(kTvrThreads) void k_try_velrot_rw2(TvrArgs a) {
    tvr_rw2_body<GREC>(a, blockIdx.z, blockIdx.x, threadIdx.x);
}
#endif

#ifndef EDGEHIP_TVR2_WAVES
#define EDGEHIP_TVR2_WAVES 0
#endif
template <bool PROCJF, bool GREC>
__global__ __launch_bounds__(kTvrThreads)
#if EDGEHIP_TVR2_WAVES > 0
__attribute__((amdgpu_waves_per_eu(EDGEHIP_TVR2_WAVES, EDGEHIP_TVR2_WAVES)))
#endif
void k_try_velrot2(TvrArgs a) {
    tvr2_body<PROCJF, GREC>(a, blockIdx.z, blockIdx.x, threadIdx.x);
}

__device__ __noinline__ void jacobi_eig6(const double Ain[36], double V[36], double e[6], double *A ) {
#pragma nounroll
    for (int i = 0; i < 36; i++) { A[i] = Ain[i]; V[i] = 0; }
#pragma nounroll
    for (int i = 0; i < 6; i++) V[i * 7] = 1;
    for (int sweep = 0; sweep < 30; sweep++) {
        double off = 0, diag = 0;
#pragma nounroll
        for (int p = 0; p < 6; p++) {
            diag += A[p * 7] * A[p * 7];
#pragma nounroll
            for (int q = p + 1; q < 6; q++) off += A[p * 6 + q] * A[p * 6 + q];
        }
        if (!(off > 1e-32 * diag) || !(off > 0)) break;
#pragma nounroll
        for (int p = 0; p < 5; p++)
#pragma nounroll
            for (int q = p + 1; q < 6; q++) {
                const double apq = A[p * 6 + q];
                if (apq == 0) continue;
                const double theta = (A[q * 7] - A[p * 7]) / (2 * apq);
                const double t = (theta >= 0 ? 1.0 : -1.0) / (fabs(theta) + sqrt(theta * theta + 1));
                const double c = 1 / sqrt(t * t + 1), s = t * c;
#pragma nounroll
                for (int k = 0; k < 6; k++) {
                    const double akp = A[k * 6 + p], akq = A[k * 6 + q];
                    A[k * 6 + p] = c * akp - s * akq;
                    A[k * 6 + q] = s * akp + c * akq;
                }
#pragma nounroll
                for (int k = 0; k < 6; k++) {
                    const double apk = A[p * 6 + k], aqk = A[q * 6 + k];
                    A[p * 6 + k] = c * apk - s * aqk;
                    A[q * 6 + k] = s * apk + c * aqk;
                }
#pragma nounroll
                for (int k = 0; k < 6; k++) {
                    const double vkp = V[k * 6 + p], vkq = V[k * 6 + q];
                    V[k * 6 + p] = c * vkp - s * vkq;
                    V[k * 6 + q] = s * vkp + c * vkq;
                }
            }
    }
#pragma nounroll
    for (int i = 0; i < 6; i++) e[i] = A[i * 7];
}

__device__ __noinline__ void svd_backsub6(const double A[36], const double b[6], double h[6], double *V, double *Awork,
                                          double *e, double *y) {
    jacobi_eig6(A, V, e, Awork);
    double smax = 0;
#pragma nounroll
    for (int i = 0; i < 6; i++) smax = fmax(smax, fabs(e[i]));
#pragma nounroll
    for (int i = 0; i < 6; i++) {
        double d = 0;
#pragma nounroll
        for (int k = 0; k < 6; k++) d += V[k * 6 + i] * b[k];
        const double inv = (fabs(e[i]) * 1e9 <= smax) ? 0.0 : 1.0 / e[i];
        y[i] = d * inv;
    }
#pragma nounroll
    for (int k = 0; k < 6; k++) {
        double d = 0;
#pragma nounroll
        for (int i = 0; i < 6; i++) d += V[k * 6 + i] * y[i];
        h[k] = d;
    }
}

__device__ __noinline__ void chol6(const double A[36], double L[36]) {
#pragma nounroll
    for (int i = 0; i < 36; i++) L[i] = A[i];
#pragma nounroll
    for (int col = 0; col < 6; col++) {
        double inv_diag = 1;
#pragma nounroll
        for (int row = col; row < 6; row++) {
            double val = L[row * 6 + col];
#pragma nounroll
            for (int col2 = 0; col2 < col; col2++) val -= L[col2 * 6 + col] * L[row * 6 + col2];
// ... 115 lines not shown
            for (int j = i + 1; j < 6; j++) val -= L[j * 6 + i] * r[j];
            r[i] = val;
        }
#pragma unroll
        for (int i = 0; i < 6; i++) Inv[i * 6 + c] = r[i];
    }
}

__device__ __forceinline__ void lm_solve6(const double (&ApI)[36], const double (&nb)[6], const bool svd_rule, double (&hh)[6],
                                          double (*s_m)[36], double (*s_v)[6]) {
    double L[36];
    chol6_r(ApI, L);
    bool use_svd = false;
    if (svd_rule) {
        double dmin = L[0], tr = ApI[0];
#pragma unroll
        for (int i = 1; i < 6; i++) { dmin = fmin(dmin, L[i * 7]); tr += ApI[i * 7]; }
        double bound = 1;
#pragma unroll
        for (int i = 0; i < 6; i++) bound *= tr / L[i * 7];
        use_svd = !(dmin > 0) || !(bound < 0.99e9);
    }
    if (use_svd) {
        double *A_l = s_m[0], *b_l = s_v[0], *h_l = s_v[2] + 0;
        for (int i = 0; i < 36; i++) A_l[i] = ApI[i];
        for (int i = 0; i < 6; i++) b_l[i] = nb[i];
        svd_backsub6(A_l, b_l, h_l, s_m[2], s_m[3], s_v[1], s_m[1]);
#pragma unroll
        for (int i = 0; i < 6; i++) hh[i] = h_l[i];
    } else {
        chol6_backsub_r(L, nb, hh);
    }
}

__global__ __launch_bounds__(64) void k_lm_solve(const double *__restrict__ A, const double *__restrict__ b, double *__restrict__ h,
                                                  int svd_rule) {
    __shared__ double s_m[4][36], s_v[3][6];
    if (threadIdx.x != 0) return;
    double ApI[36], nb[6], hh[6];
    for (int i = 0; i < 36; i++) ApI[i] = A[(size_t)blockIdx.x * 36 + i];
    for (int i = 0; i < 6; i++) nb[i] = b[(size_t)blockIdx.x * 6 + i];
    lm_solve6(ApI, nb, svd_rule != 0, hh, s_m, s_v);
    for (int i = 0; i < 6; i++) h[(size_t)blockIdx.x * 6 + i] = hh[i];
}

enum LmOps : unsigned {
    LM_REDUCE_CUR = 1u << 0,
    LM_REDUCE_NEW = 1u << 1,
    LM_NOJAC = 1u << 2,
    LM_INIT = 1u << 3,
    LM_RESET_V = 1u << 4,
    LM_GAIN_RATIO = 1u << 5,
    LM_GAIN_DIFF = 1u << 6,
    LM_SWAP_ON_ACCEPT = 1u << 7,
    LM_SAVE_T = 1u << 8,
    LM_PICK = 1u << 9,
    LM_SOLVE_SVD = 1u << 10,
    LM_SOLVE_CHOL = 1u << 11,
    LM_SETUP_X = 1u << 12,
    LM_SETUP_XNEW = 1u << 13,
    LM_FINISH = 1u << 14,
    LM_BEGIN = 1u << 15,
    LM_PHASE_A = 1u << 16,
    LM_PHASE_BC = 1u << 17,
    LM_BEGIN_KF = 1u << 18,
    LM_FINISH_KF = 1u << 19,
    LM_BEGIN2 = 1u << 20,
    LM_PICK2 = 1u << 21,
};

struct LmArgs {
    SeqDev *seq;
    const double *partials;
    const double *block_last;
    const double *partials_z = nullptr, *block_last_z = nullptr;
    double *resid_carry;
    uint32_t *framecount;
    int nblk, nseq;
    unsigned ops;
    int init_type;
    const edgehip_kf_request *kf_in;
    edgehip_kf_result *kf_out;
    const int32_t *kn_src = nullptr;
    int f32 = 0;
};
__device__ __forceinline__ double lm_rt(const double x, const int f32) { return f32 ? (double)(float)x : x; }

template <bool WAVE_ONLY>
__device__ __forceinline__ void lm_sync() {
    if (WAVE_ONLY) {
        __builtin_amdgcn_fence(__ATOMIC_SEQ_CST, "workgroup");
        __builtin_amdgcn_wave_barrier();
    } else {
        __syncthreads();
    }
}

template <bool WAVE_ONLY, bool DUAL = false>
__device__ __forceinline__ void lm_body(const LmArgs &a, const int seq, const int tid) {
    static_assert(!(WAVE_ONLY && DUAL), "the two chains meet at workgroup barriers");
    constexpr int NT = DUAL ? 128 : 64;
    const int lane = tid & 63;
    const int ch = DUAL ? tid >> 6 : 0;
    const unsigned ops = a.ops;
    static_assert(sizeof(SeqDev) % 8 == 0, "SeqDev is copied as 64-bit words");
    constexpr int kWords = sizeof(SeqDev) / 8;
    __shared__ unsigned long long s_state[kWords];
    unsigned long long *gstate = reinterpret_cast<unsigned long long *>(a.seq + seq);
    const double *a_partials = ch ? a.partials_z : a.partials;
    const double *a_block_last = ch ? a.block_last_z : a.block_last;
    constexpr int kPre = 32;
    const bool prefetch = a.nblk <= 2 * kPre && (ops & (LM_REDUCE_CUR | LM_REDUCE_NEW));
    const int pv_v = lane & 31, pv_g = lane >> 5;
    const bool pv_on = pv_v < kNumSums && (!(ops & LM_NOJAC) || pv_v == kNumSums - 1);
    double pv[kPre];
    double bl_pre = 0;
    if (prefetch) {
        const double *pp = a_partials + (size_t)seq * a.nblk * kNumSums;
#pragma unroll
        for (int j = 0; j < kPre; j++) {
            const int b = pv_g + 2 * j;
            pv[j] = (pv_on && b < a.nblk) ? pp[(size_t)b * kNumSums + pv_v] : 0.0;
        }
        if (lane < a.nblk) bl_pre = a_block_last[(size_t)seq * a.nblk + lane];
    }
    for (int i = tid; i < kWords; i += NT) s_state[i] = gstate[i];
    lm_sync<WAVE_ONLY>();
    SeqDev *sq = reinterpret_cast<SeqDev *>(s_state);
    if (a.kn_src) {
        if (tid == 0) sq->kn_old = a.kn_src[seq];
        lm_sync<WAVE_ONLY>();
    }
    const int kn = sq->kn_old;
    if (ops & LM_BEGIN) {
        if (tid == 0) {
            sq->eff_steps = 0;
            sq->v = 2;
            sq->res_cur = 0; sq->res_new = 1; sq->res_t = 2;
            sq->pub.minimizer_evals = 0;
            if (ops & LM_BEGIN2) {
                for (int i = 0; i < 6; i++) sq->zX[i] = 0;
                sq->z_eff_steps = 0;
                sq->zv = 2;
                for (int i = 0; i < 3; i++) { sq->X[i] = lm_rt(sq->pub.V[i], a.f32); sq->X[3 + i] = lm_rt(sq->pub.W[i], a.f32); }
            } else if (a.init_type == 1) {
                for (int i = 0; i < 3; i++) { sq->X[i] = lm_rt(sq->pub.V[i], a.f32); sq->X[3 + i] = lm_rt(sq->pub.W[i], a.f32); }
            } else {
                for (int i = 0; i < 6; i++) sq->X[i] = 0;
            }
            sq->s_rho_min_eval = sq->pub.s_rho_q;
        }
        lm_sync<WAVE_ONLY>();
    }
    if (ops & LM_BEGIN_KF) {
        if (lane == 0) {
            sq->eff_steps = 0;
            sq->v = 2;
            sq->res_cur = 0; sq->res_new = 1; sq->res_t = 2;
            sq->pub.minimizer_evals = 0;
            for (int i = 0; i < 6; i++) sq->X[i] = a.kf_in[seq].X0[i];
            sq->s_rho_min_eval = a.kf_in[seq].max_s_rho;
        }
        lm_sync<WAVE_ONLY>();
    }
    if (kn <= 0 && (ops & LM_FINISH_KF) && lane == 0) {
        edgehip_kf_result &o = a.kf_out[seq];
        for (int i = 0; i < 6; i++) o.X[i] = a.kf_in[seq].X0[i];
        for (int i = 0; i < 36; i++) o.RRV[i] = 0;
        o.score_ratio = 0; o.F = 0; o.F0 = 0; o.evals = 0; o.mnum = 0;
    }
    if (kn <= 0) {
        for (int i = tid; i < kWords; i += NT) gstate[i] = s_state[i];
        return;
    }
    const int nblk_used = (kn + kTvrBlock - 1) / kTvrBlock;

    constexpr int NCH = DUAL ? 2 : 1;
    __shared__ double s_part_[NCH][2][32];
    __shared__ double s_m_[NCH][4][36], s_v_[NCH][3][6];
    __shared__ double s_sum_[NCH][kNumSums];
    __shared__ double s_bl_[NCH][256];
    double (*s_part)[32] = s_part_[ch];
    double (*s_m)[36] = s_m_[ch];
    double (*s_v)[6] = s_v_[ch];
    double *s_sum = s_sum_[ch], *s_bl = s_bl_[ch];
    double *cX = ch ? sq->zX : sq->X, *cXnew = ch ? sq->zXnew : sq->Xnew, *ch_h = ch ? sq->zh : sq->h;
    double *cJtJ = ch ? sq->zJtJ : sq->JtJ, *cJtF = ch ? sq->zJtF : sq->JtF;
    double *cJtJnew = ch ? sq->zJtJnew : sq->JtJnew, *cJtFnew = ch ? sq->zJtFnew : sq->JtFnew;
    double *cF = ch ? &sq->zF : &sq->F, *cFnew = ch ? &sq->zFnew : &sq->Fnew, *cF0 = ch ? &sq->zF0 : &sq->F0;
    double *cu = ch ? &sq->zu : &sq->u, *cv = ch ? &sq->zv : &sq->v, *cgain = ch ? &sq->zgain : &sq->gain;
    int32_t *c_eff = ch ? &sq->z_eff_steps : &sq->eff_steps;
    if (ops & (LM_REDUCE_CUR | LM_REDUCE_NEW)) {
        const double *pp = a_partials + (size_t)seq * a.nblk * kNumSums;
        const int v = lane & 31, g = lane >> 5;
        double acc = 0;
        if (prefetch) {
#pragma unroll
            for (int j = 0; j < kPre; j++)
                if (g + 2 * j < nblk_used) acc += pv[j];
        } else if (v < kNumSums && (!(ops & LM_NOJAC) || v == kNumSums - 1)) {
#pragma unroll 8
            for (int b = g; b < nblk_used; b += 2) acc += pp[(size_t)b * kNumSums + v];
        }
        s_part[g][v] = acc;
        const int res_out = DUAL ? (ch ? sq->res_t : sq->res_new) : (sq->lm_phase == 0 ? sq->res_t : sq->res_new);
        double *cr = a.resid_carry + ((size_t)res_out * a.nseq + seq) * a.nblk;
        const double *bl = a_block_last + (size_t)seq * a.nblk;
        if (prefetch) {
            const bool valid = lane < nblk_used && !is_carry(bl_pre);
            const unsigned long long vm = __ballot(valid);
            const unsigned long long below = vm & ((1ull << lane) - 1ull);
            const int src = below ? 63 - __clzll(below) : 0;
            const double inh = __shfl(bl_pre, src, 64);
            if (lane < nblk_used) cr[lane] = below ? inh : 0.0;
        } else {
            for (int b = lane; b < nblk_used; b += 64) s_bl[b & 255] = bl[b];
        }
        lm_sync<WAVE_ONLY>();
        if (lane < kNumSums) {
            double t = 0;
            t = s_part[0][lane] + s_part[1][lane];
            s_sum[lane] = t;
        }
        if (!prefetch && lane == 32) {
            double run = 0;
            for (int b = 0; b < nblk_used; b++) {
                cr[b] = run;
                const double v2 = nblk_used <= 256 ? s_bl[b] : bl[b];
                if (!is_carry(v2)) run = v2;
            }
        }
    }
    lm_sync<WAVE_ONLY>();
    if (lane == 0) {
    double JtJ[36], JtF[6], X[6], Xn[6], hh[6];
#pragma unroll
    for (int i = 0; i < 36; i++) JtJ[i] = cJtJ[i];
#pragma unroll
    for (int i = 0; i < 6; i++) { JtF[i] = cJtF[i]; X[i] = cX[i]; Xn[i] = cXnew[i]; hh[i] = ch_h[i]; }
    double F = *cF, Fnew = *cFnew, F0 = *cF0, u = *cu, v = *cv;
    int eff_steps = *c_eff, res_cur = sq->res_cur, res_new = sq->res_new, res_t = sq->res_t;

    if (ops & (LM_REDUCE_CUR | LM_REDUCE_NEW)) {
        double Jn[36], Fn6[6];
        if (!(ops & LM_NOJAC)) {
            {
                int ns = 0;
#pragma unroll
                for (int i = 0; i < 6; i++)
#pragma unroll
                    for (int j = i; j < 6; j++) Jn[i * 6 + j] = lm_rt(s_sum[ns++], a.f32);
#pragma unroll
                for (int i = 0; i < 6; i++) Fn6[i] = lm_rt(s_sum[ns++], a.f32);
            }
#pragma unroll
            for (int i = 0; i < 2; i++) {
                Fn6[i + 2] = -Fn6[i + 2];
#pragma unroll
// ... 555 lines not shown
    }
    EH_LAUNCH_CHECK();
    hipLaunchKernelGGL(k_field_to16, dim3((unsigned)((pl.f16stride + 255) / 256), 1, pl.nseq), dim3(256), 0, c->stream, c->field,
                       c->field16, pl.w, pl.h, pl.fstride, pl.ftx, pl.f16stride, pl.f16tx);
    c->field32_valid = true;
    EH_LAUNCH_CHECK();
    return 0;
}

int tvr_prepare_enqueue(edgehip_ctx *c, int slot_old, unsigned begin_ops) {
    ProfScope ps(c, PROF_B_PREP);
    const DevicePlan &pl = c->plan;
    if (begin_ops) {
        LmArgs l;
        l.seq = c->seq; l.partials = c->partials; l.block_last = c->block_last; l.resid_carry = c->resid_carry;
        l.framecount = c->framecount + (size_t)c->fc_index * pl.nseq;
        l.nblk = c->nblk_tvr; l.nseq = pl.nseq; l.ops = begin_ops; l.init_type = c->p.tracker_init_type;
        l.kf_in = c->kf_req_dev; l.kf_out = c->kf_res_dev;
        l.kn_src = c->kn_slot + (size_t)slot_old * pl.nseq;
        l.f32 = c->tracker_f32 ? 1 : 0;
        hipLaunchKernelGGL(k_tvr_prepare_begin, dim3((pl.cap + 255) / 256, 1, pl.nseq), dim3(256), 0, c->stream, l.kn_src, c->resid,
                           c->resid_carry, pl.cap, c->nblk_tvr, l);
        EH_LAUNCH_CHECK();
        return 0;
    }
    hipLaunchKernelGGL(k_tvr_prepare, dim3((pl.cap + 255) / 256, 1, pl.nseq), dim3(256), 0, c->stream, kldev(c, slot_old),
                       c->kn_slot + (size_t)slot_old * pl.nseq, c->P0, c->resid, c->resid_carry, c->seq, pl.cap,
                       c->nblk_tvr, pl.zfm);
    EH_LAUNCH_CHECK();
    return 0;
}

static TvrArgs make_tvr_args(edgehip_ctx *c, int slot_new, int slot_old, double match_thresh, double k_huber,
                             uint32_t match_num_thresh, int write_mid) {
    const DevicePlan &pl = c->plan;
    TvrArgs a;
    a.kl_old = kldev(c, slot_old); a.kl_new = kldev(c, slot_new);
    a.kn_old = c->kn_slot + (size_t)slot_old * pl.nseq;
    a.field16 = c->field16; a.f16stride = pl.f16stride; a.f16tx = pl.f16tx; a.P0 = c->P0; a.resid = c->resid; a.resid_carry = c->resid_carry;
    a.block_last = c->block_last; a.partials = c->partials; a.seq = c->seq;
    a.block_last_z = c->block_last + (size_t)pl.nseq * c->nblk_tvr;
    a.partials_z = c->partials + (size_t)pl.nseq * c->nblk_tvr * kNumSums;
    a.framecount = c->framecount + (size_t)c->fc_index * pl.nseq;
    a.w = pl.w; a.h = pl.h; a.cap = pl.cap; a.nblk = c->nblk_tvr; a.nseq = pl.nseq;
    a.zfm = pl.zfm; a.inv_zfm = 1.0 / pl.zfm; a.max_r = (double)c->field_radius; a.match_thresh = match_thresh; a.k_huber = k_huber; a.inv_k_huber = 1.0 / k_huber;
    a.ppx = pl.ppx; a.ppy = pl.ppy; a.match_num_thresh = match_num_thresh; a.write_mid = write_mid;
    a.use_grec = c->grec_ok[slot_new] && !c->no_grec;
    a.kf = nullptr; a.kf_match_mod = a.kf_match_cang = a.kf_rho_tol = 0;
    a.fwd_key = (write_mid && c->fwd_key_in_tvr) ? c->fwd_key : nullptr;
    return a;
}

static int launch_tvr(edgehip_ctx *c, const TvrArgs &a, bool reweight, bool procjf) {
    ProfScope ps(c, PROF_B_TRYVELROT);
    dim3 g(c->nblk_tvr, 1, c->plan.nseq), b(kTvrThreads);
#ifdef EDGEHIP_EXPERIMENTS
    if (reweight && procjf && c->tvr_rw2 && (size_t)c->nblk_tvr * c->plan.nseq >= (size_t)c->tvr_rw2) {
        dim3 g2((c->nblk_tvr + 1) / 2, 1, c->plan.nseq);
        if (a.use_grec) hipLaunchKernelGGL((k_try_velrot_rw2<true>), g2, b, 0, c->stream, a);
        else hipLaunchKernelGGL((k_try_velrot_rw2<false>), g2, b, 0, c->stream, a);
        EH_LAUNCH_CHECK();
        return 0;
    }
#endif
#ifdef EDGEHIP_EXPERIMENTS
    static const size_t dyn_lds = getenv("EDGEHIP_TVR_LDS") ? (size_t)atoi(getenv("EDGEHIP_TVR_LDS")) : 0;
#else
    constexpr size_t dyn_lds = 0;
#endif
    if (c->tracker_f32) {
#define EH_TVF(RW, JF)                                                                                                   \
    do {                                                                                                                 \
        if (a.use_grec) hipLaunchKernelGGL((k_try_velrot_f32<RW, JF, true>), g, b, 0, c->stream, a);                      \
        else hipLaunchKernelGGL((k_try_velrot_f32<RW, JF, false>), g, b, 0, c->stream, a);                                \
    } while (0)
        if (reweight && procjf) EH_TVF(true, true);
        else if (reweight) EH_TVF(true, false);
        else if (procjf) EH_TVF(false, true);
        else EH_TVF(false, false);
#undef EH_TVF
        EH_LAUNCH_CHECK();
        return 0;
    }
    if (a.use_grec) {
        if (reweight && procjf) hipLaunchKernelGGL((k_try_velrot<true, true, true>), g, b, dyn_lds, c->stream, a);
        else if (reweight) hipLaunchKernelGGL((k_try_velrot<true, false, true>), g, b, dyn_lds, c->stream, a);
        else if (procjf) hipLaunchKernelGGL((k_try_velrot<false, true, true>), g, b, dyn_lds, c->stream, a);
        else hipLaunchKernelGGL((k_try_velrot<false, false, true>), g, b, dyn_lds, c->stream, a);
    } else {
        if (reweight && procjf) hipLaunchKernelGGL((k_try_velrot<true, true, false>), g, b, dyn_lds, c->stream, a);
        else if (reweight) hipLaunchKernelGGL((k_try_velrot<true, false, false>), g, b, dyn_lds, c->stream, a);
        else if (procjf) hipLaunchKernelGGL((k_try_velrot<false, true, false>), g, b, dyn_lds, c->stream, a);
        else hipLaunchKernelGGL((k_try_velrot<false, false, false>), g, b, dyn_lds, c->stream, a);
    }
    EH_LAUNCH_CHECK();
    return 0;
}

static int launch_lm(edgehip_ctx *c, int slot_new, unsigned ops, bool two_chains = false) {
    ProfScope ps(c, PROF_B_LMSTEP);
    LmArgs a;
    a.seq = c->seq; a.partials = c->partials; a.block_last = c->block_last; a.resid_carry = c->resid_carry;
    a.block_last_z = c->block_last + (size_t)c->plan.nseq * c->nblk_tvr;
    a.partials_z = c->partials + (size_t)c->plan.nseq * c->nblk_tvr * kNumSums;
    a.framecount = c->framecount + (size_t)c->fc_index * c->plan.nseq;
    a.nblk = c->nblk_tvr; a.nseq = c->plan.nseq; a.ops = ops; a.init_type = c->p.tracker_init_type;
    a.kf_in = c->kf_req_dev; a.kf_out = c->kf_res_dev;
    a.f32 = c->tracker_f32 ? 1 : 0;
    if (two_chains) hipLaunchKernelGGL(k_lm_step2, dim3(c->plan.nseq), dim3(128), 0, c->stream, a);
    else hipLaunchKernelGGL(k_lm_step, dim3(c->plan.nseq), dim3(64), 0, c->stream, a);
    EH_LAUNCH_CHECK();
    return 0;
}

static int launch_tvr2(edgehip_ctx *c, const TvrArgs &a, bool procjf) {
    ProfScope ps(c, PROF_B_TRYVELROT2);
    dim3 g(c->nblk_tvr, 1, c->plan.nseq), b(kTvrThreads);
    if (c->tracker_f32) {
        if (a.use_grec) {
            if (procjf) hipLaunchKernelGGL((k_try_velrot2_f32<true, true>), g, b, 0, c->stream, a);
            else hipLaunchKernelGGL((k_try_velrot2_f32<false, true>), g, b, 0, c->stream, a);
        } else {
            if (procjf) hipLaunchKernelGGL((k_try_velrot2_f32<true, false>), g, b, 0, c->stream, a);
            else hipLaunchKernelGGL((k_try_velrot2_f32<false, false>), g, b, 0, c->stream, a);
        }
        EH_LAUNCH_CHECK();
        return 0;
    }
    if (a.use_grec) {
        if (procjf) hipLaunchKernelGGL((k_try_velrot2<true, true>), g, b, 0, c->stream, a);
        else hipLaunchKernelGGL((k_try_velrot2<false, true>), g, b, 0, c->stream, a);
    } else {
        if (procjf) hipLaunchKernelGGL((k_try_velrot2<true, false>), g, b, 0, c->stream, a);
        else hipLaunchKernelGGL((k_try_velrot2<false, false>), g, b, 0, c->stream, a);
    }
    EH_LAUNCH_CHECK();
    return 0;
}

__global__ __launch_bounds__(256) void k_count_forward(const KlSoA *kls, const int32_t *__restrict__ kns, edgehip_kf_result *out) {
    __shared__ int s_n[4];
    const int seq = blockIdx.x, kn = kns[seq];
    int n = 0;
    for (int i = threadIdx.x; i < kn; i += 256) n += kls[seq].m_id_f[i] >= 0;
#pragma unroll
    for (int o = 32; o > 0; o >>= 1) n += __shfl_xor(n, o, 64);
    if ((threadIdx.x & 63) == 0) s_n[threadIdx.x >> 6] = n;
    __syncthreads();
    if (threadIdx.x == 0) out[seq].mnum = s_n[0] + s_n[1] + s_n[2] + s_n[3];
}

int minimizer_kf_enqueue(edgehip_ctx *c, int slot_kf, int slot_cur, double match_mod, double match_ang, double rho_tol, int iter_max,
                         double reweight_distance, uint32_t match_num_thresh) {
    int e;
    c->fc_index = slot_kf;
#define EH_TRY(x) if ((e = (x)) != 0) return e
    EH_TRY(rec_refresh_enqueue(c, slot_kf));
    EH_TRY(tvr_prepare_enqueue(c, slot_cur));
    auto eval = [&](bool last) -> int {
        TvrArgs a = make_tvr_args(c, slot_kf, slot_cur, 0.0, reweight_distance, match_num_thresh, last ? 1 : 0);
        a.kf = c->kf_req_dev; a.kf_match_mod = match_mod; a.kf_match_cang = cos(match_ang); a.kf_rho_tol = rho_tol;
        a.use_grec = 0;
        ProfScope ps(c, PROF_B_TRYVELROT);
        hipLaunchKernelGGL(k_try_velrot_kf, dim3(c->nblk_tvr, 1, c->plan.nseq), dim3(kTvrThreads), 0, c->stream, a);
        EH_LAUNCH_CHECK();
        return 0;
    };
    const int M = iter_max;
    EH_TRY(launch_lm(c, slot_kf, LM_BEGIN_KF | LM_SETUP_X | LM_PHASE_BC));
    EH_TRY(eval(M <= 0));
    {
        unsigned ops = LM_REDUCE_CUR | LM_INIT | LM_RESET_V;
        if (M > 0) ops |= LM_SOLVE_CHOL | LM_SETUP_XNEW; else ops |= LM_FINISH_KF;
        EH_TRY(launch_lm(c, slot_kf, ops));
    }
    for (int it = 0; it < M; it++) {
        EH_TRY(eval(it == M - 1));
        unsigned ops = LM_REDUCE_NEW | LM_GAIN_RATIO | LM_SWAP_ON_ACCEPT;
        if (it < M - 1) ops |= LM_SOLVE_CHOL | LM_SETUP_XNEW; else ops |= LM_FINISH_KF;
        EH_TRY(launch_lm(c, slot_kf, ops));
    }
    hipLaunchKernelGGL(k_count_forward, dim3(c->plan.nseq), dim3(256), 0, c->stream, kldev(c, slot_cur),
                       c->kn_slot + (size_t)slot_cur * c->plan.nseq, c->kf_res_dev);
    EH_LAUNCH_CHECK();
#undef EH_TRY
    return 0;
}

int minimizer_enqueue(edgehip_ctx *c, int slot_new, int slot_old, int fc_index) {
    const edgehip_params &p = c->p;
    c->fc_index = fc_index;
    int e;
    if ((e = rec_refresh_enqueue(c, slot_new))) return e;
    const bool fuse = c->persist_lm_max > 0 && c->plan.nseq <= c->persist_lm_max;
    const bool two_chains = p.tracker_init_type >= 2 && c->dual_init && !fuse;
    const unsigned begin_ops = two_chains ? (LM_BEGIN | LM_BEGIN2 | LM_SETUP_X | LM_PHASE_BC)
                                          : (LM_BEGIN | LM_SETUP_X | (p.tracker_init_type >= 2 ? LM_PHASE_A : LM_PHASE_BC));
    const bool begin_rides = c->plan.nseq <= 64;
    if ((e = tvr_prepare_enqueue(c, slot_old, begin_rides ? begin_ops : 0u))) return e;
    if (!begin_rides && (e = edgehip::launch_lm(c, slot_new, begin_ops))) return e;
    if (c->fwd_key_in_tvr && !c->fwd_cleared) EH_CHECK(hipMemsetAsync(c->fwd_key, 0, sizeof(unsigned long long) * (size_t)c->plan.nseq * c->plan.cap, c->stream));
    const int I = p.tracker_init_iter_num, M = p.tracker_iter_num;
    const int total_evals = (p.tracker_init_type >= 2 ? 2 * (1 + (I > 0 ? I : 0)) : 0) + 1 + (M > 0 ? M : 0);
    int evals = 0;
    struct { bool on, rw, jf; int write_mid; } held = {false, false, false, 0};
    auto eval = [&](bool rw, bool jf) -> int {
        evals++;
        if (fuse) {
            held = {true, rw, jf, evals == total_evals};
            return 0;
        }
        TvrArgs a = make_tvr_args(c, slot_new, slot_old, p.tracker_match_thresh, p.reweight_distance, p.match_num_thresh,
                                  evals == total_evals);
        return launch_tvr(c, a, rw, jf);
    };
    auto launch_lm = [&](edgehip_ctx *cc, int sn, unsigned ops) -> int {
        if (!held.on) return edgehip::launch_lm(cc, sn, ops);
#ifndef EDGEHIP_EXPERIMENTS
        set_error("minimizer: the fused evaluation + step launch is an EXPERIMENTS build option");
        return EDGEHIP_ERR_STATE;
#else
        held.on = false;
        ProfScope ps(c, PROF_B_MINIMIZER);
        TvrArgs a = make_tvr_args(c, slot_new, slot_old, p.tracker_match_thresh, p.reweight_distance, p.match_num_thresh, held.write_mid);
        LmArgs l;
        l.seq = c->seq; l.partials = c->partials; l.block_last = c->block_last; l.resid_carry = c->resid_carry;
        l.framecount = c->framecount + (size_t)c->fc_index * c->plan.nseq;
        l.nblk = c->nblk_tvr; l.nseq = c->plan.nseq; l.ops = ops; l.init_type = c->p.tracker_init_type;
        l.kf_in = nullptr; l.kf_out = nullptr;
        dim3 g(c->nblk_tvr, 1, c->plan.nseq), b(kTvrThreads);
#define EH_TVLM(RW, JF)                                                                                                     \
    do {                                                                                                                   \
        if (a.use_grec) hipLaunchKernelGGL((k_try_velrot_lm<RW, JF, true>), g, b, 0, c->stream, a, l, c->sync_cnt);        \
        else hipLaunchKernelGGL((k_try_velrot_lm<RW, JF, false>), g, b, 0, c->stream, a, l, c->sync_cnt);                  \
    } while (0)
        if (held.rw && held.jf) EH_TVLM(true, true);
        else if (held.rw) EH_TVLM(true, false);
        else if (held.jf) EH_TVLM(false, true);
        else EH_TVLM(false, false);
#undef EH_TVLM
        EH_LAUNCH_CHECK();
        return 0;
#endif
    };
#define EH_TRY(x) if ((e = (x)) != 0) return e
    if (two_chains) {
        auto eval2 = [&](bool jf) -> int {
            evals += 2;
            TvrArgs a = make_tvr_args(c, slot_new, slot_old, p.tracker_match_thresh, p.reweight_distance, p.match_num_thresh, 0);
            return launch_tvr2(c, a, jf);
        };
        EH_TRY(eval2(true));
        unsigned ops = LM_REDUCE_CUR | LM_INIT | LM_RESET_V;
        ops |= I > 0 ? (LM_SOLVE_SVD | LM_SETUP_XNEW) : (LM_PICK2 | LM_SETUP_X);
        EH_TRY(edgehip::launch_lm(c, slot_new, ops, true));
        for (int i = 0; i < I; i++) {
            const bool last = (i == I - 1);
            EH_TRY(eval2(!last));
            ops = LM_REDUCE_NEW | (last ? (LM_NOJAC | LM_GAIN_DIFF) : LM_GAIN_RATIO);
            ops |= !last ? (LM_SOLVE_SVD | LM_SETUP_XNEW) : (LM_PICK2 | LM_SETUP_X);
            EH_TRY(edgehip::launch_lm(c, slot_new, ops, true));
        }
    } else if (p.tracker_init_type >= 2) {
        for (int trial = 0; trial < 2; trial++) {
            const unsigned phase = trial == 0 ? LM_PHASE_A : LM_PHASE_BC;
            (void)phase;
            EH_TRY(eval(false, true));
            unsigned ops = LM_REDUCE_CUR | LM_INIT | (trial == 1 ? LM_RESET_V : 0);
            if (I > 0) ops |= LM_SOLVE_SVD | LM_SETUP_XNEW;
            unsigned tail = trial == 0 ? (LM_SAVE_T | LM_SETUP_X | LM_PHASE_BC) : (LM_PICK | LM_SETUP_X);
            if (I <= 0) ops |= tail;
            EH_TRY(launch_lm(c, slot_new, ops));
            for (int i = 0; i < I; i++) {
                const bool last = (i == I - 1);
                EH_TRY(eval(false, !last));
                ops = LM_REDUCE_NEW | (last ? (LM_NOJAC | LM_GAIN_DIFF) : LM_GAIN_RATIO);
                if (!last) ops |= LM_SOLVE_SVD | LM_SETUP_XNEW;
                else ops |= tail;
                EH_TRY(launch_lm(c, slot_new, ops));
            }
        }
    }
    EH_TRY(eval(true, true));
    {
        unsigned ops = LM_REDUCE_CUR | LM_INIT | LM_RESET_V;
        if (M > 0) ops |= LM_SOLVE_CHOL | LM_SETUP_XNEW; else ops |= LM_FINISH;
        EH_TRY(launch_lm(c, slot_new, ops));
    }
    for (int it = 0; it < M; it++) {
        EH_TRY(eval(true, true));
        unsigned ops = LM_REDUCE_NEW | LM_GAIN_RATIO | LM_SWAP_ON_ACCEPT;
        if (it < M - 1) ops |= LM_SOLVE_CHOL | LM_SETUP_XNEW; else ops |= LM_FINISH;
        EH_TRY(launch_lm(c, slot_new, ops));
    }
#undef EH_TRY
    return 0;
}

int minimizer_v_enqueue(edgehip_ctx *c, int slot_new, int slot_old, int fc_index, int iter_max, double match_thresh,
                        uint32_t match_num_thresh, double reweight_distance) {
    const DevicePlan &pl = c->plan;
    c->fc_index = fc_index;
    const int nblk256 = (pl.cap + 255) / 256;
    if (nblk256 > c->nblk_tvr * (kTvrBlock / 256)) { set_error("minimizer_v: block tables too small"); return EDGEHIP_ERR_STATE; }
    static_assert(kTvrBlock == 256, "k_try_vel shares the per-block tables of k_try_velrot");
    if (int e = rec_refresh_enqueue(c, slot_new)) return e;
    EH_CHECK(hipMemsetAsync(c->resid, 0, sizeof(double) * pl.nseq * pl.cap, c->stream));
    TvrArgs a = make_tvr_args(c, slot_new, slot_old, match_thresh, reweight_distance, match_num_thresh, 1);
    a.fwd_key = nullptr;
    c->fwd_keys_posted = c->fwd_cleared;
    const int32_t *kn_old = c->kn_slot + (size_t)slot_old * pl.nseq;
    auto eval = [&](bool use_new, bool last) {
        dim3 g(nblk256, 1, pl.nseq), b(256);
        TvrArgs al = a;
        if (last && c->fwd_keys_posted) al.fwd_key = c->fwd_key;
        if (use_new) hipLaunchKernelGGL((k_try_vel<true>), g, b, 0, c->stream, al);
        else hipLaunchKernelGGL((k_try_vel<false>), g, b, 0, c->stream, al);
    };
    auto step = [&](unsigned ops) {
        hipLaunchKernelGGL(k_lmv_step, dim3(pl.nseq), dim3(64), 0, c->stream, c->seq, c->partials, c->block_last, c->resid_carry,
                           kn_old, c->nblk_tvr, ops);
        if ((ops & (LMV_REDUCE_CUR | LMV_REDUCE_NEW)) && (ops & LMV_FINISH))
            hipLaunchKernelGGL(k_tv_resolve, dim3(nblk256, 1, pl.nseq), dim3(256), 0, c->stream, c->resid, c->resid_carry, kn_old,
                               pl.cap, c->nblk_tvr);
    };
    eval(false, iter_max <= 0);
    step(LMV_BEGIN | LMV_REDUCE_CUR | (iter_max > 0 ? LMV_SOLVE : LMV_FINISH));
    for (int it = 0; it < iter_max; it++) {
        eval(true, it == iter_max - 1);
        step(LMV_REDUCE_NEW | LMV_GAIN | (it < iter_max - 1 ? LMV_SOLVE : LMV_FINISH));
    }
    EH_LAUNCH_CHECK();
    return 0;
}

}

using namespace edgehip;

extern "C" {

int edgehip_quantile(edgehip_ctx *c, int slot, double a, double b, double pct, int n) {
    EH_ENTER(c);
    if (!c || slot < 0 || slot >= c->plan.nslots) return EDGEHIP_ERR_ARG;
// ... 84 lines not shown

int edgehip_download_resid(edgehip_ctx *c, int which, double *resid) {
    EH_ENTER(c);
    if (!c || !resid || which < 0 || which >= kResidBufs) return EDGEHIP_ERR_ARG;
    const DevicePlan &pl = c->plan;
    hipLaunchKernelGGL(k_resolve_resid, dim3((pl.cap + 255) / 256, 1, pl.nseq), dim3(256), 0, c->stream,
                       c->resid + (size_t)which * pl.nseq * pl.cap, c->resid_carry + (size_t)which * pl.nseq * c->nblk_tvr,
                       c->rs_tmp, pl.cap, c->nblk_tvr);
    EH_LAUNCH_CHECK();
    EH_CHECK(hipMemcpyAsync(resid, c->rs_tmp, sizeof(double) * pl.nseq * pl.cap, hipMemcpyDeviceToHost, c->stream));
    EH_CHECK(hipStreamSynchronize(c->stream));
    return 0;
}

int edgehip_minimizer_v(edgehip_ctx *c, int slot_new, int slot_old, double *V, const double *s_rho_min, float min_mod,
                        double match_thresh, int iter_max, uint32_t match_num_thresh, double reweight_distance, double *RVel,
                        double *F) {
    EH_ENTER(c);
    if (!c || !V || !s_rho_min || slot_new < 0 || slot_old < 0 || slot_new >= c->plan.nslots || slot_old >= c->plan.nslots ||
        iter_max < 0) {
        set_error("minimizer_v: bad argument");
        return EDGEHIP_ERR_ARG;
    }
    if (int e = rot_materialize_enqueue(c, slot_old)) return e;
    const int B = c->plan.nseq;
    EH_CHECK(hipMemcpyAsync(c->pinned_seq, c->seq, sizeof(SeqDev) * B, hipMemcpyDeviceToHost, c->stream));
    EH_CHECK(hipStreamSynchronize(c->stream));
    for (int s = 0; s < B; s++) {
        SeqDev &q = c->pinned_seq[s];
        for (int i = 0; i < 3; i++) q.mv_V[i] = V[s * 3 + i];
        q.mv_s_rho_min = s_rho_min[s];
        q.mv_min_mod = min_mod < 0.f ? 0.f : min_mod;
    }
    EH_CHECK(hipMemcpyAsync(c->seq, c->pinned_seq, sizeof(SeqDev) * B, hipMemcpyHostToDevice, c->stream));
    if (min_mod < 0.f) {
        std::vector<float> rt(B);
        EH_CHECK(hipMemcpyAsync(rt.data(), c->retuned_slot + (size_t)slot_old * B, sizeof(float) * B, hipMemcpyDeviceToHost, c->stream));
        EH_CHECK(hipStreamSynchronize(c->stream));
        for (int s = 0; s < B; s++) c->pinned_seq[s].mv_min_mod = rt[s];
        EH_CHECK(hipMemcpyAsync(c->seq, c->pinned_seq, sizeof(SeqDev) * B, hipMemcpyHostToDevice, c->stream));
    }
    if (int e = minimizer_v_enqueue(c, slot_new, slot_old, slot_new, iter_max, match_thresh, match_num_thresh, reweight_distance)) return e;
    EH_CHECK(hipMemcpyAsync(c->pinned_seq, c->seq, sizeof(SeqDev) * B, hipMemcpyDeviceToHost, c->stream));
    EH_CHECK(hipStreamSynchronize(c->stream));
    for (int s = 0; s < B; s++) {
        const SeqDev &q = c->pinned_seq[s];
        for (int i = 0; i < 3; i++) V[s * 3 + i] = q.mv_V[i];
        if (RVel) for (int i = 0; i < 9; i++) RVel[s * 9 + i] = q.mv_RVel[i];
        if (F) F[s] = q.mv_F;
    }
    return 0;
}

int edgehip_minimizer_rv_kf(edgehip_ctx *c, int slot_kf, int slot_cur, const edgehip_kf_request *req, double match_mod, double match_ang,
                            double rho_tol, int iter_max, double reweight_distance, uint32_t match_num_thresh, edgehip_kf_result *res) {
    EH_ENTER(c);
    if (!c || !req || !res || slot_kf < 0 || slot_cur < 0 || slot_kf >= c->plan.nslots || slot_cur >= c->plan.nslots || slot_kf == slot_cur)
        return EDGEHIP_ERR_ARG;
    const size_t B = c->plan.nseq;
    if (!c->kf_req_dev) {
        void *q = nullptr;
        if (hipMalloc(&q, sizeof(edgehip_kf_request) * B) != hipSuccess) { (void)hipGetLastError(); set_error("kf request alloc failed"); return EDGEHIP_ERR_MEMORY; }
        c->kf_req_dev = (edgehip_kf_request *)q;
        if (hipMalloc(&q, sizeof(edgehip_kf_result) * B) != hipSuccess) { (void)hipGetLastError(); set_error("kf result alloc failed"); return EDGEHIP_ERR_MEMORY; }
        c->kf_res_dev = (edgehip_kf_result *)q;
    }
    if (int e = rot_materialize_enqueue(c, slot_cur)) return e;
    if (int e = sync_all(c)) return e;
    EH_CHECK(hipMemcpy(c->kf_req_dev, req, sizeof(edgehip_kf_request) * B, hipMemcpyHostToDevice));
    if (int e = build_field_enqueue(c, slot_kf, c->p.search_range, -1.f)) return e;
    if (int e = minimizer_kf_enqueue(c, slot_kf, slot_cur, match_mod, match_ang, rho_tol, iter_max, reweight_distance, match_num_thresh)) return e;
    EH_CHECK(hipStreamSynchronize(c->stream));
    EH_CHECK(hipMemcpy(res, c->kf_res_dev, sizeof(edgehip_kf_result) * B, hipMemcpyDeviceToHost));
    return 0;
}

int edgehip_minimizer_rv(edgehip_ctx *c, int slot_new, int slot_old) {
    EH_ENTER(c);
    if (!c || slot_new < 0 || slot_old < 0 || slot_new >= c->plan.nslots || slot_old >= c->plan.nslots) return EDGEHIP_ERR_ARG;
    if (int e = rot_materialize_enqueue(c, slot_old)) return e;
    return minimizer_enqueue(c, slot_new, slot_old, slot_new);
}

}
```

### rebvo_amd/edgehip.py

```python
import ctypes as C
import os

import numpy as np

HERE = os.path.dirname(os.path.abspath(__file__))
LIB_PATH = os.path.join(HERE, "lib", "libedgehip.so")

KEYLINE_DTYPE = np.dtype(
    [
        ("p_inx", "<i4"), ("m_m", "<f4", (2,)), ("u_m", "<f4", (2,)), ("n_m", "<f4"), ("score", "<f4"),
        ("c_p", "<f4", (2,)), ("_pad0", "<i4"),
        ("rho", "<f8"), ("s_rho", "<f8"), ("rho_nr", "<f8"), ("s_rho_nr", "<f8"), ("rho0", "<f8"), ("s_rho0", "<f8"),
        ("p_m", "<f4", (2,)), ("p_m_0", "<f4", (2,)),
        ("m_id", "<i4"), ("m_id_f", "<i4"), ("m_id_kf", "<i4"), ("m_num", "<i4"),
        ("m_m0", "<f4", (2,)), ("n_m0", "<f8"),
        ("p_id", "<i4"), ("n_id", "<i4"), ("net_id", "<i4"), ("stereo_m_id", "<i4"),
        ("stereo_rho", "<f8"), ("stereo_s_rho", "<f8"),
    ]
)
assert KEYLINE_DTYPE.itemsize == 168

NET_KEYLINE_DTYPE = np.dtype({"names": ["qx", "qy", "rho", "s_rho", "n_kl", "m_num", "flow"],
                              "formats": ["<u2", "<u2", "<u2", "<u2", "<i4", "u1", ("u1", (2,))],
                              "offsets": [0, 2, 4, 6, 8, 12, 13], "itemsize": 15})
# ... 152 lines not shown
class NavImu(C.Structure):
    _fields_ = [("Rot", C.c_double * 9), ("RotLie", C.c_double * 3), ("RotGiro", C.c_double * 3), ("Vel", C.c_double * 3),
                ("Pose", C.c_double * 9), ("PoseLie", C.c_double * 3), ("Pos", C.c_double * 3), ("g", C.c_double * 3),
                ("scale", C.c_double), ("dt", C.c_double), ("K", C.c_double), ("Kp", C.c_double), ("RKp", C.c_double),
                ("s_rho_q", C.c_double), ("Vg", C.c_double * 3), ("Bg", C.c_double * 3), ("dVv", C.c_double * 3),
                ("dWv", C.c_double * 3), ("Vgv", C.c_double * 3), ("Vgva", C.c_double * 3), ("Av", C.c_double * 3),
                ("As", C.c_double * 3), ("X", C.c_double * 7), ("b_est", C.c_double * 3), ("u_est", C.c_double * 3),
                ("kn", C.c_int32), ("klm_num", C.c_int32), ("estimation_ok", C.c_int32), ("init", C.c_int32)]


class DepthFillParams(C.Structure):
    _fields_ = [("block_w", C.c_int32), ("block_h", C.c_int32), ("iter_num", C.c_int32), ("thresh_rel_rho", C.c_double),
                ("thresh_match_num", C.c_int32), ("bound_mode", C.c_int32), ("discard", C.c_int32)]


class DepthSurfaceParams(C.Structure):
    _fields_ = [("surface", C.c_int32), ("image_mode", C.c_int32)]


class SurfaceViewsParams(C.Structure):
    _fields_ = [("capacity", C.c_int32), ("nx", C.c_int32), ("ny", C.c_int32), ("nz", C.c_int32)]


class KfPose(C.Structure):
    _fields_ = [("t", C.c_double), ("K", C.c_double), ("Rot", C.c_double * 9), ("RotLie", C.c_double * 3), ("Vel", C.c_double * 3),
                ("Pose", C.c_double * 9), ("PoseLie", C.c_double * 3), ("Pos", C.c_double * 3)]


class KfTrack(C.Structure):
    _fields_ = [("fow_m0", C.c_int32), ("fow_m", C.c_int32), ("back_m0", C.c_int32), ("back_m", C.c_int32),
                ("inserted", C.c_int32), ("kf_count", C.c_int32), ("guard", C.c_int32), ("kf_kn", C.c_int32)]


class KfListInfo(C.Structure):
    _fields_ = [("kf_count", C.c_int32), ("first", C.c_int32), ("held", C.c_int32), ("overwritten", C.c_int32)]


KF_POSE_DTYPE = np.dtype(KfPose)
KF_TRACK_DTYPE = np.dtype(KfTrack)
KF_LIST_INFO_DTYPE = np.dtype(KfListInfo)


class KfPairCount(C.Structure):
    _fields_ = [("kl_on_fov", C.c_int32), ("kl_match", C.c_int32), ("kls_on_fov", C.c_int32), ("guard", C.c_int32)]


class KfCovisArgs(C.Structure):
    _fields_ = [("field_radius", C.c_int32), ("field_min_mod", C.c_float), ("match_mod", C.c_float), ("match_ang", C.c_float),
                ("rho_tol", C.c_float), ("max_r", C.c_float)]


KF_PAIR_COUNT_DTYPE = np.dtype(KfPairCount)
assert KF_PAIR_COUNT_DTYPE.itemsize == 16 and C.sizeof(KfCovisArgs) == 24


class KfConstraintArgs(C.Structure):
    _fields_ = [("direction", C.c_int32), ("iter_max", C.c_int32), ("k_huber", C.c_double)]


class KfConstraint(C.Structure):
    _fields_ = [("X", C.c_double * 6), ("W_X", C.c_double * 36), ("R_X", C.c_double * 36),
                ("ratio", C.c_double), ("E", C.c_double), ("E0", C.c_double), ("Kp", C.c_double), ("W_Kp", C.c_double),
                ("links", C.c_int32), ("inliers", C.c_int32), ("evals", C.c_int32), ("accepted", C.c_int32), ("guard", C.c_int32),
                ("pad", C.c_int32)]


KF_CONSTRAINT_DTYPE = np.dtype(KfConstraint)
assert KF_CONSTRAINT_DTYPE.itemsize == 688 and C.sizeof(KfConstraintArgs) == 16


class KfDepth(C.Structure):
    _fields_ = [("count", C.c_int32), ("guard", C.c_int32), ("K", C.c_double), ("rTr", C.c_double), ("rTr0", C.c_double)]


KF_DEPTH_DTYPE = np.dtype(KfDepth)
assert KF_DEPTH_DTYPE.itemsize == 32
NAV_DTYPE = np.dtype(Nav)
assert NAV_DTYPE.itemsize == C.sizeof(Nav)

EXPORTS = [
    "edgehip_create", "edgehip_destroy", "edgehip_last_error", "edgehip_abi_version", "edgehip_sync",
    "edgehip_stream", "edgehip_box_widths", "edgehip_upload_rgb", "edgehip_upload_rgb_device",
    "edgehip_stage_a", "edgehip_get_kn", "edgehip_quantile", "edgehip_build_field", "edgehip_try_velrot",
    "edgehip_download_resid", "edgehip_minimizer_rv", "edgehip_forward_match", "edgehip_rotate_keylines",
    "edgehip_directed_matching", "edgehip_regularize_ekf", "edgehip_rescale", "edgehip_process_frame",
    "edgehip_next_slot", "edgehip_cur_slot", "edgehip_read_nav", "edgehip_reset", "edgehip_get_state",
    "edgehip_set_state", "edgehip_get_framecount", "edgehip_set_framecount", "edgehip_download_keylines", "edgehip_download_keylines_batch",
    "edgehip_upload_keylines", "edgehip_download_plane", "edgehip_download_field", "edgehip_profile_enable",
    "edgehip_profile_count", "edgehip_profile_name", "edgehip_profile_read", "edgehip_profile_select",
    "edgehip_upload_rgb_indexed", "edgehip_bind_rgb_indexed", "edgehip_set_nav_log", "edgehip_read_nav_log", "edgehip_read_nav_log_device", "edgehip_read_nav_imu_log", "edgehip_read_stereo_matches_log", "edgehip_set_tracker_precision", "edgehip_export_keylines", "edgehip_export_fetch", "edgehip_export_wait",
    "edgehip_build_undistort_map", "edgehip_download_undistorted", "edgehip_depth_reset", "edgehip_depth_reset_slot", "edgehip_set_slot_camera", "edgehip_directed_matching_stereo",
    "edgehip_alloc_pinned", "edgehip_free_pinned", "edgehip_upload_rgb_pinned", "edgehip_upload_sync", "edgehip_upload_wait", "edgehip_register_host", "edgehip_unregister_host", "edgehip_experiments", "edgehip_fuse_stereo_depth", "edgehip_set_stereo_rig", "edgehip_get_stereo_matches", "edgehip_minimizer_v", "edgehip_ext_rot_vel",
    "edgehip_imu_enable", "edgehip_set_imu", "edgehip_read_nav_imu", "edgehip_minimizer_rv_kf", "edgehip_lm_solve",
    "edgehip_upload_grey8", "edgehip_upload_grey8_pinned", "edgehip_bind_grey8_indexed",
    "edgehip_depth_fill_enable", "edgehip_depth_fill_size", "edgehip_depth_fill", "edgehip_download_depth_grid",
    "edgehip_download_depth_grids_batch",
    "edgehip_depth_surface_enable", "edgehip_depth_surface", "edgehip_download_depth_surface", "edgehip_download_depth_surfaces_batch",
    "edgehip_download_depth_image", "edgehip_download_depth_images_batch", "edgehip_depth_image_device",
    "edgehip_surface_views_enable", "edgehip_surface_view_capture", "edgehip_surface_view_upload", "edgehip_surface_view_clear",
    "edgehip_surface_space", "edgehip_surface_integrate", "edgehip_download_surface_visibility",
    "edgehip_download_surface_visibilities_batch", "edgehip_surface_ray_cross",
    "edgehip_net_enable", "edgehip_net_pack", "edgehip_download_net_keylines", "edgehip_download_net_keylines_batch",
    "edgehip_net_keylines_device", "edgehip_upload_net_keylines", "edgehip_depth_fill_net",
    "edgehip_ros_enable", "edgehip_ros_pack", "edgehip_download_ros_edgemap", "edgehip_download_ros_edgemaps_batch",
    "edgehip_ros_edgemap_device", "edgehip_ros_edgemap_from_device", "edgehip_ros_export", "edgehip_ros_export_fetch", "edgehip_ros_export_wait",
    "edgehip_match_one_pass",
    "edgehip_keyframe_track_enable", "edgehip_keyframe_insert", "edgehip_keyframe_build_forward_match", "edgehip_keyframe_forward_correct",
    "edgehip_keyframe_back_correct", "edgehip_read_keyframe_track", "edgehip_download_keyframe", "edgehip_upload_keyframe",
    "edgehip_keyframe_set_save", "edgehip_keyframe_list_enable", "edgehip_keyframe_list_info", "edgehip_download_keyframe_list",
    "edgehip_download_keyframe_list_batch", "edgehip_keyframe_list_restore",
    "edgehip_keyframe_covisibility", "edgehip_keyframe_covisibility_slot", "edgehip_keyframe_covisibility_ms",
    "edgehip_keyframe_constraint", "edgehip_keyframe_mutual_exclusion", "edgehip_keyframe_constraint_ms",
    "edgehip_keyframe_map_depth", "edgehip_keyframe_translate_depth", "edgehip_keyframe_list_translate_depth", "edgehip_keyframe_depth_ms",
    "edgehip_keyframe_depth_select",
]

_lib = None


def load_library():
    global _lib
    if _lib is None:
        if not os.path.exists(LIB_PATH):
            raise RuntimeError(f"{LIB_PATH} is missing: build it with `make -C rebvo_amd/csrc` "
                               "(or __graft_entry__.build()); rebvo_amd has no CPU fallback")
        _lib = C.CDLL(LIB_PATH)
        _lib.edgehip_last_error.restype = C.c_char_p
        _lib.edgehip_profile_name.restype = C.c_char_p
        _lib.edgehip_stream.restype = C.c_void_p
    return _lib


class EdgeHipError(RuntimeError):
    pass


def build_undistort_map(params):
    lib = load_library()
    n = params.w * params.h
    inx, iw = np.empty((n, 4), np.int32), np.empty((n, 4), np.int32)
    rc = lib.edgehip_build_undistort_map(C.byref(params), C.c_void_p(inx.ctypes.data), C.c_void_p(iw.ctypes.data))
    if rc != 0:
        raise EdgeHipError(f"edgehip_build_undistort_map: {rc}")
    return inx, iw


def _dp(a):
    return a.ctypes.data_as(C.POINTER(C.c_double))


KF_FILE_CAM_DTYPE = np.dtype([("pp", "<f4", (2,)), ("zf", "<f4", (2,)), ("zfm", "<f8"), ("Kc", "<f8", (5,)), ("w", "<i4"), ("h", "<i4")])
assert KF_FILE_CAM_DTYPE.itemsize == 72 and KF_POSE_DTYPE.itemsize == 256


def keyframe_file_camera(params):
    cam = np.zeros((), KF_FILE_CAM_DTYPE)
    cam["pp"] = (params.ppx, params.ppy)
    cam["zf"] = (params.zfx, params.zfy)
    cam["zfm"] = np.float32((cam["zf"][0] + cam["zf"][1]) / np.float32(2))
    cam["Kc"] = list(params.kc)
    cam["w"], cam["h"] = params.w, params.h
    return cam


def write_keyframe_file(path, keyframes, params, max_r=None):
    cam = keyframe_file_camera(params)
    max_r = float(params.search_range if max_r is None else max_r)
# ... 179 lines not shown
        assert idx.shape == (self.nseq,)
        self._ck(self.lib.edgehip_upload_rgb_indexed(self.ctx, slot, C.c_void_p(pool_dev_ptr), pool_frames,
                                                     idx.ctypes.data_as(C.c_void_p)))

    def set_tracker_precision(self, bits):
        self._ck(self.lib.edgehip_set_tracker_precision(self.ctx, bits))

    def set_nav_log(self, length):
        self._ck(self.lib.edgehip_set_nav_log(self.ctx, length))

    def read_nav_log(self, first, count):
        out = (Nav * (count * self.nseq))()
        self._ck(self.lib.edgehip_read_nav_log(self.ctx, first, count, out))
        return [[out[k * self.nseq + s] for s in range(self.nseq)] for k in range(count)]

    def read_nav_log_array(self, first, count):
        out = np.zeros((count, self.nseq), dtype=NAV_DTYPE)
        self._ck(self.lib.edgehip_read_nav_log(self.ctx, first, count, out.ctypes.data_as(C.c_void_p)))
        return out

    def read_nav_imu_log(self, first, count):
        out = (NavImu * (count * self.nseq))()
        self._ck(self.lib.edgehip_read_nav_imu_log(self.ctx, first, count, out))
        return [[out[k * self.nseq + s] for s in range(self.nseq)] for k in range(count)]

    def read_stereo_matches_log(self, first, count):
        out = np.zeros((count, self.nseq), dtype=np.int32)
        self._ck(self.lib.edgehip_read_stereo_matches_log(self.ctx, first, count, out.ctypes.data_as(C.c_void_p)))
        return out

    def read_nav_log_device(self, first, count, out_dev_ptr):
        self._ck(self.lib.edgehip_read_nav_log_device(self.ctx, first, count, C.c_void_p(out_dev_ptr)))

    def sync(self):
        self._ck(self.lib.edgehip_sync(self.ctx))

    def stream(self):
        return self.lib.edgehip_stream(self.ctx)

    def box_widths(self):
        out = (C.c_int * 6)()
        self._ck(self.lib.edgehip_box_widths(self.ctx, out))
        return list(out)

    def stage_a(self, slot):
        self._ck(self.lib.edgehip_stage_a(self.ctx, slot))

    def get_kn(self, slot):
        out = np.zeros(self.nseq, np.int32)
        self._ck(self.lib.edgehip_get_kn(self.ctx, slot, out.ctypes.data_as(C.c_void_p)))
        return out

    def quantile(self, slot, smin=1e-3, smax=20.0, pct=0.9, nbins=100):
        self._ck(self.lib.edgehip_quantile(self.ctx, slot, C.c_double(smin), C.c_double(smax), C.c_double(pct), nbins))

    def build_field(self, slot, radius, min_mod=-1.0):
        self._ck(self.lib.edgehip_build_field(self.ctx, slot, radius, C.c_float(min_mod)))

    def try_velrot(self, slot_new, slot_old, X, reweight, procjf, match_thresh, s_rho_min, match_num_thresh, k_huber,
                   resid_in=-1, resid_out=0):
        X = np.ascontiguousarray(np.broadcast_to(np.asarray(X, np.float64), (self.nseq, 6)))
        smin = np.ascontiguousarray(np.broadcast_to(np.asarray(s_rho_min, np.float64), (self.nseq,)))
        out = np.zeros((self.nseq, 43))
        self._ck(self.lib.edgehip_try_velrot(self.ctx, slot_new, slot_old, _dp(X), int(reweight), int(procjf),
                                             C.c_double(match_thresh), _dp(smin), C.c_uint32(match_num_thresh),
                                             C.c_double(k_huber), resid_in, resid_out, _dp(out)))
        return out[:, 42].copy(), out[:, :36].reshape(self.nseq, 6, 6).copy(), out[:, 36:42].copy()

    def download_resid(self, which):
        out = np.zeros((self.nseq, self.cap))
        self._ck(self.lib.edgehip_download_resid(self.ctx, which, _dp(out)))
        return out

    def lm_solve(self, A, b, svd_rule):
        A = np.ascontiguousarray(A, np.float64).reshape(-1, 36)
        b = np.ascontiguousarray(b, np.float64).reshape(-1, 6)
        h = np.zeros_like(b)
        self._ck(self.lib.edgehip_lm_solve(self.ctx, _dp(A), _dp(b), len(A), int(bool(svd_rule)), _dp(h)))
        return h

    def minimizer_rv(self, slot_new, slot_old):
        self._ck(self.lib.edgehip_minimizer_rv(self.ctx, slot_new, slot_old))

    def forward_match(self, slot_old, slot_new):
        self._ck(self.lib.edgehip_forward_match(self.ctx, slot_old, slot_new))

    def rotate_keylines(self, slot, R=None):
        if R is None:
            self._ck(self.lib.edgehip_rotate_keylines(self.ctx, slot, None))
        else:
            R = np.ascontiguousarray(np.broadcast_to(np.asarray(R, np.float64).reshape(-1, 9), (self.nseq, 9)))
            self._ck(self.lib.edgehip_rotate_keylines(self.ctx, slot, _dp(R)))

    def directed_matching(self, slot_new, slot_old):
        self._ck(self.lib.edgehip_directed_matching(self.ctx, slot_new, slot_old))

    def match_one_pass(self, slot_new, slot_old, fill=False):
        self._ck(self.lib.edgehip_match_one_pass(self.ctx, slot_new, slot_old, int(bool(fill))))

    def regularize_ekf(self, slot, do_regularize=True, do_ekf=True):
        self._ck(self.lib.edgehip_regularize_ekf(self.ctx, slot, int(do_regularize), int(do_ekf)))

    def rescale(self, slot):
        self._ck(self.lib.edgehip_rescale(self.ctx, slot))

    def next_slot(self):
        return self.lib.edgehip_next_slot(self.ctx)

    def cur_slot(self):
        return self.lib.edgehip_cur_slot(self.ctx)

    def alloc_pinned_frames(self, count=None):
        count = self.nseq if count is None else count
        nbytes = count * self.h * self.w * 3
        ptr = C.c_void_p()
        self._ck(self.lib.edgehip_alloc_pinned(C.c_size_t(nbytes), C.byref(ptr)))
        buf = (C.c_uint8 * nbytes).from_address(ptr.value)
        arr = np.frombuffer(buf, np.uint8).reshape(count, self.h, self.w, 3)
        return arr, ptr

    def free_pinned(self, ptr):
        self._ck(self.lib.edgehip_free_pinned(ptr))

    def upload_rgb_pinned(self, slot, ptr, seq_first=0, count=None):
        self._ck(self.lib.edgehip_upload_rgb_pinned(self.ctx, slot, ptr, seq_first, self.nseq if count is None else count))

    def process_frame(self, t):
        t = np.ascontiguousarray(np.broadcast_to(np.asarray(t, np.float64), (self.nseq,)))
        self._ck(self.lib.edgehip_process_frame(self.ctx, _dp(t)))

    def read_nav(self):
        nav = (Nav * self.nseq)()
        self._ck(self.lib.edgehip_read_nav(self.ctx, nav))
        return list(nav)

    def imu_enable(self, imu_params):
        self._ck(self.lib.edgehip_imu_enable(self.ctx, C.byref(imu_params)))

    def set_imu(self, records):
        arr = (ImuIntegrated * self.nseq)(*records)
        self._ck(self.lib.edgehip_set_imu(self.ctx, arr))

    def read_nav_imu(self):
        out = (NavImu * self.nseq)()
        self._ck(self.lib.edgehip_read_nav_imu(self.ctx, out))
        return list(out)

    def reset(self):
        self._ck(self.lib.edgehip_reset(self.ctx))

    def get_state(self, seq=0):
        s = SeqState()
        self._ck(self.lib.edgehip_get_state(self.ctx, seq, C.byref(s)))
        return s

    def set_state(self, seq, s):
        self._ck(self.lib.edgehip_set_state(self.ctx, seq, C.byref(s)))

    def get_framecount(self, seq, slot):
        v = C.c_uint32(0)
        self._ck(self.lib.edgehip_get_framecount(self.ctx, seq, slot, C.byref(v)))
        return v.value

    def set_framecount(self, seq, slot, fc):
        self._ck(self.lib.edgehip_set_framecount(self.ctx, seq, slot, C.c_uint32(fc)))

# ... 559 lines not shown
```

Before: 132,700.

## Compact tracker keylines into a keep list before velocity-rotation evaluations

Adds a per-sequence prepass kernel that scans the old keylines once, marks the gated-out ones, and writes a compacted index list (with skipped zero-rho entries tagged by bitwise complement) plus its count. The try_velrot evaluation kernels and the LM step then iterate only over the compacted list, so each LM iteration launches fewer blocks and skips the per-keyline gate test. Residual buffers are indexed by list position instead of keyline index. The cost is one extra kernel launch per minimizer call and an indirection load per thread, and the gate is now evaluated once rather than per evaluation.

```diff
diff --git a/include/edgehip.h b/include/edgehip.h
--- a/include/edgehip.h
+++ b/include/edgehip.h
@@ -134,6 +134,7 @@
                        int resid_in, int resid_out, double *out);
 int edgehip_download_resid(edgehip_ctx *ctx, int which, double *resid);
 int edgehip_minimizer_rv(edgehip_ctx *ctx, int slot_new, int slot_old);
+int edgehip_read_keep_counts(edgehip_ctx *ctx, int32_t *nk, int32_t *kn);
 int edgehip_set_tracker_precision(edgehip_ctx *ctx, int bits);
 int edgehip_lm_solve(edgehip_ctx *ctx, const double *A, const double *b, int n, int svd_rule, double *h);
 
diff --git a/rebvo_amd/csrc/api.hip b/rebvo_amd/csrc/api.hip
--- a/rebvo_amd/csrc/api.hip
+++ b/rebvo_amd/csrc/api.hip
@@ -460,6 +460,8 @@
     EH_TRY(dmalloc(c, &c->resid_carry, (size_t)kResidBufs * B * c->nblk_tvr, al->dev, 0));
     EH_TRY(dmalloc(c, &c->partials, 2 * B * c->nblk_tvr * kNumSums, al->dev, 0));
     EH_TRY(dmalloc(c, &c->block_last, 2 * B * c->nblk_tvr, al->dev, 0));
+    EH_TRY(dmalloc(c, &c->keep, B * CAP, al->dev, 0));
+    EH_TRY(dmalloc(c, &c->keep_n, B, al->dev, 0));
     EH_TRY(dmalloc(c, &c->bin_cnt, B * 256, al->dev, 0));
     {
         const size_t ntiles = (size_t)((p.w + 63) / 64) * ((p.h + 63) / 64);
diff --git a/rebvo_amd/csrc/ctx.h b/rebvo_amd/csrc/ctx.h
--- a/rebvo_amd/csrc/ctx.h
+++ b/rebvo_amd/csrc/ctx.h
@@ -372,6 +372,8 @@
     double *resid_carry;
     double *partials;
     double *block_last;
+    int32_t *keep;
+    int32_t *keep_n;
     bool use_graph;
     std::map<int, hipGraphExec_t> frame_graphs;
     struct StereoRig {
diff --git a/rebvo_amd/csrc/stage_b.hip b/rebvo_amd/csrc/stage_b.hip
--- a/rebvo_amd/csrc/stage_b.hip
+++ b/rebvo_amd/csrc/stage_b.hip
@@ -509,6 +509,74 @@
     resid0[(size_t)seq * cap + i] = 0.0;
 }
 
+constexpr int kKeepThreads = 1024, kKeepTurns = 16;
+__global__ __launch_bounds__(kKeepThreads) void k_tvr_prepare_keep(const KlSoA *kls, const int32_t *__restrict__ kns, const SeqDev *seqs,
+                                                                   const uint32_t *__restrict__ framecount, uint32_t match_num_thresh,
+                                                                   int32_t *__restrict__ keep, int32_t *__restrict__ keep_n, int cap) {
+    constexpr int NW = kKeepThreads / 64;
+    static_assert(kKeepTurns * NW == 256, "wave 0 scans four counts per lane");
+    const int seq = blockIdx.x, tid = threadIdx.x, lane = tid & 63, wave = tid >> 6;
+    const int kn = kns[seq] < cap ? kns[seq] : cap;
+    const KlSoA &ko = kls[seq];
+    const double gate = seqs[seq].pub.s_rho_q;
+    const uint32_t fc = framecount[seq];
+    const uint32_t mthr = match_num_thresh < fc ? match_num_thresh : fc;
+    int32_t *out = keep + (size_t)seq * cap;
+    __shared__ int s_cnt[kKeepTurns * NW];
+    __shared__ int s_total;
+    const unsigned long long below = (1ull << lane) - 1ull;
+    int base = 0;
+    for (int i0 = 0; i0 < kn; i0 += kKeepTurns * kKeepThreads) {
+        double sr[kKeepTurns];
+        int32_t mn[kKeepTurns];
+#pragma unroll
+        for (int it = 0; it < kKeepTurns; it++) {
+            const int ikl = i0 + it * kKeepThreads + tid;
+            sr[it] = ikl < kn ? ldg(ko.s_rho, ikl) : 0.0;
+            mn[it] = ikl < kn ? ldg(ko.m_num, ikl) : 0;
+        }
+        unsigned listed_m = 0, skip_m = 0;
+#pragma unroll
+        for (int it = 0; it < kKeepTurns; it++) {
+            const int ikl = i0 + it * kKeepThreads + tid;
+            const bool skip = ikl < kn && (sr[it] > gate || (uint32_t)mn[it] < mthr);
+            const bool listed = ikl < kn && (!skip || sr[it] == 0);
+            if (skip) stg(ko.m_id_f, ikl, -1);
+            listed_m |= (unsigned)listed << it;
+            skip_m |= (unsigned)skip << it;
+            const unsigned long long m = __ballot(listed);
+            if (lane == 0) s_cnt[it * NW + wave] = __popcll(m);
+        }
+        __syncthreads();
+        if (wave == 0) {
+            int c[4], t = 0;
+#pragma unroll
+            for (int j = 0; j < 4; j++) { c[j] = s_cnt[lane * 4 + j]; t += c[j]; }
+            int incl = t;
+#pragma unroll
+            for (int o = 1; o < 64; o <<= 1) {
+                const int v = __shfl_up(incl, o, 64);
+                if (lane >= o) incl += v;
+            }
+            int run = incl - t;
+#pragma unroll
+            for (int j = 0; j < 4; j++) { s_cnt[lane * 4 + j] = run; run += c[j]; }
+            if (lane == 63) s_total = incl;
+        }
+        __syncthreads();
+#pragma unroll
+        for (int it = 0; it < kKeepTurns; it++) {
+            const int ikl = i0 + it * kKeepThreads + tid;
+            const bool listed = (listed_m >> it) & 1u;
+            const unsigned long long m = __ballot(listed);
+            if (listed) out[base + s_cnt[it * NW + wave] + __popcll(m & below)] = ((skip_m >> it) & 1u) ? ~ikl : ikl;
+        }
+        base += s_total;
+        __syncthreads();
+    }
+    if (tid == 0) keep_n[seq] = base;
+}
+
 __device__ __forceinline__ void so3_exp_inl(const double (&w)[3], double (&R)[9]) {
     const double one_6th = 1.0 / 6.0, one_20th = 1.0 / 20.0;
     const double theta_sq = w[0] * w[0] + w[1] * w[1] + w[2] * w[2];
@@ -575,6 +643,7 @@
     const KlSoA *kl_old;
     const KlSoA *kl_new;
     const int32_t *kn_old;
+    const int32_t *keep = nullptr, *keep_n = nullptr;
     const uint16_t *field16;
     const double *P0;
     double *resid;
@@ -648,12 +717,13 @@
     J[5] = (T)-1 * t0; J[5] += J[1] * ptx;
 }
 
-template <bool REWEIGHT, bool PROCJF, bool GREC, bool KF = false>
+template <bool REWEIGHT, bool PROCJF, bool GREC, bool KF = false, bool KEEP = false>
 __device__ __forceinline__ void tvr_body(const TvrArgs &a, const int seq, const int blk, const int tid) {
     constexpr int ABL = KF ? 0 : EDGEHIP_TVR_ABL;
     const int lane = tid & 63, wave = tid >> 6;
     SeqDev *sq = a.seq + seq;
-    const int kn = a.kn_old[seq];
+    static_assert(!(KF && KEEP), "the key-frame evaluation has no keep list");
+    const int kn = KEEP ? a.keep_n[seq] : a.kn_old[seq];
     if (blk * kTvrBlock >= kn) return;
     const KlSoA &ko = a.kl_old[seq];
     const int res_in = sq->res_cur, res_out = sq->lm_phase == 0 ? sq->res_t : sq->res_new;
@@ -670,7 +740,14 @@
 #pragma unroll
     for (int i = 0; i < kNumSums; i++) sums[i] = 0;
 
-    const int ikl = blk * kTvrBlock + tid;
+    const int pos = blk * kTvrBlock + tid;
+    int ikl = pos;
+    bool listed_skip = false;
+    if (KEEP && pos < kn) {
+        const int32_t e = a.keep[(size_t)seq * a.cap + pos];
+        listed_skip = e < 0;
+        ikl = e < 0 ? ~e : e;
+    }
     double J[6] = {0, 0, 0, 0, 0, 0};
     double fm, dfx, dfy;
     double ptx, pty, ptz, pix, piy, rho_p, s_rho;
@@ -683,19 +760,20 @@
     int status = 0;
     double fi = 0;
     double rho_own;
-    if (ikl < kn) {
+    if (pos < kn) {
         s_rho = ldg(ko.s_rho, ikl);
-        const int32_t mnum = ldg(ko.m_num, ikl);
+        int32_t mnum = 0;
+        if (!KEEP) mnum = ldg(ko.m_num, ikl);
         const float2 pm0 = ldg(ko.p_m, ikl);
         const double rho0 = ldg(ko.rho, ikl);
         rho_own = rho0;
         const float2 klm = ldg(ko.m_m, ikl);
         const float knm = ldg(ko.n_m, ikl);
         double rprev = 0;
-        if (REWEIGHT && !(ABL & 16)) rprev = rin[ikl];
+        if (REWEIGHT && !(ABL & 16)) rprev = rin[pos];
         const uint32_t fc = KF ? 0xFFFFFFFFu : a.framecount[seq];
         const uint32_t mthr = a.match_num_thresh < fc ? a.match_num_thresh : fc;
-        const bool skip = s_rho > sq->s_rho_min_eval || (uint32_t)mnum < mthr;
+        const bool skip = KEEP ? listed_skip : (s_rho > sq->s_rho_min_eval || (uint32_t)mnum < mthr);
         if (!skip) {
             const double sz = inv_mid(rho0);
             const double pz_zf0 = a.inv_zfm * sz;
@@ -780,16 +858,16 @@
         carry_publish(wl, lane, wave, s_wlast, s_whas);
         __syncthreads();
         if (status == 3) {
-            rout[ikl] = carry_inherit(wl, wave, s_wlast, s_whas);
+            rout[pos] = carry_inherit(wl, wave, s_wlast, s_whas);
         } else if (status == 2) {
-            rout[ikl] = fi;
+            rout[pos] = fi;
         } else if (status == 1) {
-            rout[ikl] = a.max_r;
-        } else if (ikl < kn) {
-            rout[ikl] = 0.0;
-        }
-    }
-    if (a.write_mid && ikl < kn) {
+            rout[pos] = a.max_r;
+        } else if (pos < kn) {
+            rout[pos] = 0.0;
+        }
+    }
+    if (a.write_mid && pos < kn) {
         stg(ko.m_id_f, ikl, mid_f);
         if (!KF && a.fwd_key && mid_f >= 0) atomicMax(&a.fwd_key[(size_t)seq * a.cap + mid_f], ord_bits(rho_own));
     }
@@ -823,7 +901,7 @@
         }
         fs = fm * inv_q;
 #endif
-    } else if (!REWEIGHT && !KF && ikl < kn && s_rho == 0) {
+    } else if (!REWEIGHT && !KF && pos < kn && s_rho == 0) {
         const double qnan = __longlong_as_double(0x7ff8000000000000ll);
         if (PROCJF) {
 #pragma unroll
@@ -883,9 +961,9 @@
     block_reduce_store<PROCJF>(s_red, tid, a.partials + ((size_t)seq * a.nblk + blk) * kNumSums);
 }
 
-template <bool REWEIGHT, bool PROCJF, bool GREC>
+template <bool REWEIGHT, bool PROCJF, bool GREC, bool KEEP = false>
 __global__ __launch_bounds__(kTvrThreads) void k_try_velrot(TvrArgs a) {
-    tvr_body<REWEIGHT, PROCJF, GREC>(a, blockIdx.z, blockIdx.x, threadIdx.x);
+    tvr_body<REWEIGHT, PROCJF, GREC, false, KEEP>(a, blockIdx.z, blockIdx.x, threadIdx.x);
 }
 __global__ __launch_bounds__(kTvrThreads) void k_try_velrot_kf(TvrArgs a) {
     tvr_body<true, true, false, true>(a, blockIdx.z, blockIdx.x, threadIdx.x);
@@ -1041,11 +1119,11 @@
 #ifndef EDGEHIP_TVR2_PARK
 #define EDGEHIP_TVR2_PARK 1
 #endif
-template <bool PROCJF, bool GREC>
+template <bool PROCJF, bool GREC, bool KEEP = false>
 __device__ __forceinline__ void tvr2_body(const TvrArgs &a, const int seq, const int blk, const int tid) {
     const int lane = tid & 63, wave = tid >> 6;
     SeqDev *sq = a.seq + seq;
-    const int kn = a.kn_old[seq];
+    const int kn = KEEP ? a.keep_n[seq] : a.kn_old[seq];
     if (blk * kTvrBlock >= kn) return;
     const KlSoA &ko = a.kl_old[seq];
     double *rout0 = a.resid + ((size_t)sq->res_t * a.nseq + seq) * a.cap;
@@ -1054,21 +1132,29 @@
     __shared__ double s_wlast[2][NW];
     __shared__ int s_whas[2][NW];
 
-    const int ikl = blk * kTvrBlock + tid;
+    const int pos = blk * kTvrBlock + tid;
+    int ikl = pos;
+    bool listed_skip = false;
+    if (KEEP && pos < kn) {
+        const int32_t e = a.keep[(size_t)seq * a.cap + pos];
+        listed_skip = e < 0;
+        ikl = e < 0 ? ~e : e;
+    }
     double fm[2], dfx[2], dfy[2], fi[2] = {0, 0};
     double ptx[2], pty[2], ptz[2], pix[2], piy[2], rho_p[2];
     int status[2] = {0, 0};
     double s_rho = 1;
-    if (ikl < kn) {
+    if (pos < kn) {
         s_rho = ldg(ko.s_rho, ikl);
-        const int32_t mnum = ldg(ko.m_num, ikl);
+        int32_t mnum = 0;
+        if (!KEEP) mnum = ldg(ko.m_num, ikl);
         const float2 pm0 = ldg(ko.p_m, ikl);
         const double rho0 = ldg(ko.rho, ikl);
         const float2 klm = ldg(ko.m_m, ikl);
         const float knm = ldg(ko.n_m, ikl);
         const uint32_t fc = a.framecount[seq];
         const uint32_t mthr = a.match_num_thresh < fc ? a.match_num_thresh : fc;
-        const bool skip = s_rho > sq->s_rho_min_eval || (uint32_t)mnum < mthr;
+        const bool skip = KEEP ? listed_skip : (s_rho > sq->s_rho_min_eval || (uint32_t)mnum < mthr);
         if (!skip) {
             const double sz = inv_mid(rho0);
             const double pz_zf0 = a.inv_zfm * sz;
@@ -1134,13 +1220,13 @@
     for (int c = 0; c < 2; c++) {
         double *rout = c ? rout1 : rout0;
         if (status[c] == 3) {
-            rout[ikl] = carry_inherit(wl[c], wave, s_wlast[c], s_whas[c]);
+            rout[pos] = carry_inherit(wl[c], wave, s_wlast[c], s_whas[c]);
         } else if (status[c] == 2) {
-            rout[ikl] = fi[c];
+            rout[pos] = fi[c];
         } else if (status[c] == 1) {
-            rout[ikl] = a.max_r;
-        } else if (ikl < kn) {
-            rout[ikl] = 0.0;
+            rout[pos] = a.max_r;
+        } else if (pos < kn) {
+            rout[pos] = 0.0;
         }
     }
     if (tid == 0) {
@@ -1178,7 +1264,7 @@
 #else
             fmc[c] *= inv_q;
 #endif
-        } else if (ikl < kn && s_rho == 0) {
+        } else if (pos < kn && s_rho == 0) {
             const double qnan = __longlong_as_double(0x7ff8000000000000ll);
             if (PROCJF) {
 #pragma unroll
@@ -1570,13 +1656,13 @@
 #ifndef EDGEHIP_TVR2_WAVES
 #define EDGEHIP_TVR2_WAVES 0
 #endif
-template <bool PROCJF, bool GREC>
+template <bool PROCJF, bool GREC, bool KEEP = false>
 __global__ __launch_bounds__(kTvrThreads)
 #if EDGEHIP_TVR2_WAVES > 0
 __attribute__((amdgpu_waves_per_eu(EDGEHIP_TVR2_WAVES, EDGEHIP_TVR2_WAVES)))
 #endif
 void k_try_velrot2(TvrArgs a) {
-    tvr2_body<PROCJF, GREC>(a, blockIdx.z, blockIdx.x, threadIdx.x);
+    tvr2_body<PROCJF, GREC, KEEP>(a, blockIdx.z, blockIdx.x, threadIdx.x);
 }
 
 __device__ __noinline__ void jacobi_eig6(const double Ain[36], double V[36], double e[6], double *A ) {
@@ -1858,6 +1944,7 @@
     const edgehip_kf_request *kf_in;
     edgehip_kf_result *kf_out;
     const int32_t *kn_src = nullptr;
+    const int32_t *keep_n = nullptr;
     int f32 = 0;
 };
 __device__ __forceinline__ double lm_rt(const double x, const int f32) { return f32 ? (double)(float)x : x; }
@@ -1891,6 +1978,7 @@
     const bool pv_on = pv_v < kNumSums && (!(ops & LM_NOJAC) || pv_v == kNumSums - 1);
     double pv[kPre];
     double bl_pre = 0;
+    const int nk_pre = a.keep_n ? a.keep_n[seq] : 0;
     if (prefetch) {
         const double *pp = a_partials + (size_t)seq * a.nblk * kNumSums;
 #pragma unroll
@@ -1949,7 +2037,7 @@
         for (int i = tid; i < kWords; i += NT) gstate[i] = s_state[i];
         return;
     }
-    const int nblk_used = (kn + kTvrBlock - 1) / kTvrBlock;
+    const int nblk_used = ((a.keep_n ? nk_pre : kn) + kTvrBlock - 1) / kTvrBlock;
 
     constexpr int NCH = DUAL ? 2 : 1;
     __shared__ double s_part_[NCH][2][32];
@@ -2671,22 +2759,24 @@
         EH_LAUNCH_CHECK();
         return 0;
     }
-    if (a.use_grec) {
-        if (reweight && procjf) hipLaunchKernelGGL((k_try_velrot<true, true, true>), g, b, dyn_lds, c->stream, a);
-        else if (reweight) hipLaunchKernelGGL((k_try_velrot<true, false, true>), g, b, dyn_lds, c->stream, a);
-        else if (procjf) hipLaunchKernelGGL((k_try_velrot<false, true, true>), g, b, dyn_lds, c->stream, a);
-        else hipLaunchKernelGGL((k_try_velrot<false, false, true>), g, b, dyn_lds, c->stream, a);
+#define EH_TV(GR, KP)                                                                                                    \
+    do {                                                                                                                 \
+        if (reweight && procjf) hipLaunchKernelGGL((k_try_velrot<true, true, GR, KP>), g, b, dyn_lds, c->stream, a);      \
+        else if (reweight) hipLaunchKernelGGL((k_try_velrot<true, false, GR, KP>), g, b, dyn_lds, c->stream, a);          \
+        else if (procjf) hipLaunchKernelGGL((k_try_velrot<false, true, GR, KP>), g, b, dyn_lds, c->stream, a);            \
+        else hipLaunchKernelGGL((k_try_velrot<false, false, GR, KP>), g, b, dyn_lds, c->stream, a);                       \
+    } while (0)
+    if (a.keep) {
+        if (a.use_grec) EH_TV(true, true); else EH_TV(false, true);
     } else {
-        if (reweight && procjf) hipLaunchKernelGGL((k_try_velrot<true, true, false>), g, b, dyn_lds, c->stream, a);
-        else if (reweight) hipLaunchKernelGGL((k_try_velrot<true, false, false>), g, b, dyn_lds, c->stream, a);
-        else if (procjf) hipLaunchKernelGGL((k_try_velrot<false, true, false>), g, b, dyn_lds, c->stream, a);
-        else hipLaunchKernelGGL((k_try_velrot<false, false, false>), g, b, dyn_lds, c->stream, a);
-    }
+        if (a.use_grec) EH_TV(true, false); else EH_TV(false, false);
+    }
+#undef EH_TV
     EH_LAUNCH_CHECK();
     return 0;
 }
 
-static int launch_lm(edgehip_ctx *c, int slot_new, unsigned ops, bool two_chains = false) {
+static int launch_lm(edgehip_ctx *c, int slot_new, unsigned ops, bool two_chains = false, const int32_t *keep_n = nullptr) {
     ProfScope ps(c, PROF_B_LMSTEP);
     LmArgs a;
     a.seq = c->seq; a.partials = c->partials; a.block_last = c->block_last; a.resid_carry = c->resid_carry;
@@ -2696,6 +2786,7 @@
     a.nblk = c->nblk_tvr; a.nseq = c->plan.nseq; a.ops = ops; a.init_type = c->p.tracker_init_type;
     a.kf_in = c->kf_req_dev; a.kf_out = c->kf_res_dev;
     a.f32 = c->tracker_f32 ? 1 : 0;
+    a.keep_n = keep_n;
     if (two_chains) hipLaunchKernelGGL(k_lm_step2, dim3(c->plan.nseq), dim3(128), 0, c->stream, a);
     else hipLaunchKernelGGL(k_lm_step, dim3(c->plan.nseq), dim3(64), 0, c->stream, a);
     EH_LAUNCH_CHECK();
@@ -2716,13 +2807,17 @@
         EH_LAUNCH_CHECK();
         return 0;
     }
-    if (a.use_grec) {
-        if (procjf) hipLaunchKernelGGL((k_try_velrot2<true, true>), g, b, 0, c->stream, a);
-        else hipLaunchKernelGGL((k_try_velrot2<false, true>), g, b, 0, c->stream, a);
+#define EH_TV2(GR, KP)                                                                             \
+    do {                                                                                           \
+        if (procjf) hipLaunchKernelGGL((k_try_velrot2<true, GR, KP>), g, b, 0, c->stream, a);       \
+        else hipLaunchKernelGGL((k_try_velrot2<false, GR, KP>), g, b, 0, c->stream, a);             \
+    } while (0)
+    if (a.keep) {
+        if (a.use_grec) EH_TV2(true, true); else EH_TV2(false, true);
     } else {
-        if (procjf) hipLaunchKernelGGL((k_try_velrot2<true, false>), g, b, 0, c->stream, a);
-        else hipLaunchKernelGGL((k_try_velrot2<false, false>), g, b, 0, c->stream, a);
-    }
+        if (a.use_grec) EH_TV2(true, false); else EH_TV2(false, false);
+    }
+#undef EH_TV2
     EH_LAUNCH_CHECK();
     return 0;
 }
@@ -2786,6 +2881,18 @@
     const unsigned begin_ops = two_chains ? (LM_BEGIN | LM_BEGIN2 | LM_SETUP_X | LM_PHASE_BC)
                                           : (LM_BEGIN | LM_SETUP_X | (p.tracker_init_type >= 2 ? LM_PHASE_A : LM_PHASE_BC));
     const bool begin_rides = c->plan.nseq <= 64;
+    bool use_keep = !fuse && !c->tracker_f32;
+#ifdef EDGEHIP_EXPERIMENTS
+    if (c->tvr_rw2) use_keep = false;
+#endif
+    const int32_t *keep_n = use_keep ? c->keep_n : nullptr;
+    if (use_keep) {
+        ProfScope ps(c, PROF_B_PREP);
+        hipLaunchKernelGGL(k_tvr_prepare_keep, dim3(c->plan.nseq), dim3(kKeepThreads), 0, c->stream, kldev(c, slot_old),
+                           c->kn_slot + (size_t)slot_old * c->plan.nseq, c->seq, c->framecount + (size_t)c->fc_index * c->plan.nseq,
+                           p.match_num_thresh, c->keep, c->keep_n, c->plan.cap);
+        EH_LAUNCH_CHECK();
+    }
     if ((e = tvr_prepare_enqueue(c, slot_old, begin_rides ? begin_ops : 0u))) return e;
     if (!begin_rides && (e = edgehip::launch_lm(c, slot_new, begin_ops))) return e;
     if (c->fwd_key_in_tvr && !c->fwd_cleared) EH_CHECK(hipMemsetAsync(c->fwd_key, 0, sizeof(unsigned long long) * (size_t)c->plan.nseq * c->plan.cap, c->stream));
@@ -2801,10 +2908,11 @@
         }
         TvrArgs a = make_tvr_args(c, slot_new, slot_old, p.tracker_match_thresh, p.reweight_distance, p.match_num_thresh,
                                   evals == total_evals);
+        if (use_keep) { a.keep = c->keep; a.keep_n = c->keep_n; }
         return launch_tvr(c, a, rw, jf);
     };
     auto launch_lm = [&](edgehip_ctx *cc, int sn, unsigned ops) -> int {
-        if (!held.on) return edgehip::launch_lm(cc, sn, ops);
+        if (!held.on) return edgehip::launch_lm(cc, sn, ops, false, keep_n);
 #ifndef EDGEHIP_EXPERIMENTS
         set_error("minimizer: the fused evaluation + step launch is an EXPERIMENTS build option");
         return EDGEHIP_ERR_STATE;
@@ -2837,18 +2945,19 @@
         auto eval2 = [&](bool jf) -> int {
             evals += 2;
             TvrArgs a = make_tvr_args(c, slot_new, slot_old, p.tracker_match_thresh, p.reweight_distance, p.match_num_thresh, 0);
+            if (use_keep) { a.keep = c->keep; a.keep_n = c->keep_n; }
             return launch_tvr2(c, a, jf);
         };
         EH_TRY(eval2(true));
         unsigned ops = LM_REDUCE_CUR | LM_INIT | LM_RESET_V;
         ops |= I > 0 ? (LM_SOLVE_SVD | LM_SETUP_XNEW) : (LM_PICK2 | LM_SETUP_X);
-        EH_TRY(edgehip::launch_lm(c, slot_new, ops, true));
+        EH_TRY(edgehip::launch_lm(c, slot_new, ops, true, keep_n));
         for (int i = 0; i < I; i++) {
             const bool last = (i == I - 1);
             EH_TRY(eval2(!last));
             ops = LM_REDUCE_NEW | (last ? (LM_NOJAC | LM_GAIN_DIFF) : LM_GAIN_RATIO);
             ops |= !last ? (LM_SOLVE_SVD | LM_SETUP_XNEW) : (LM_PICK2 | LM_SETUP_X);
-            EH_TRY(edgehip::launch_lm(c, slot_new, ops, true));
+            EH_TRY(edgehip::launch_lm(c, slot_new, ops, true, keep_n));
         }
     } else if (p.tracker_init_type >= 2) {
         for (int trial = 0; trial < 2; trial++) {
@@ -3099,4 +3208,15 @@
     return minimizer_enqueue(c, slot_new, slot_old, slot_new);
 }
 
-}
+int edgehip_read_keep_counts(edgehip_ctx *c, int32_t *nk, int32_t *kn) {
+    EH_ENTER(c);
+    if (!c || !nk || !kn) return EDGEHIP_ERR_ARG;
+    const int B = c->plan.nseq;
+    EH_CHECK(hipMemcpyAsync(nk, c->keep_n, sizeof(int32_t) * B, hipMemcpyDeviceToHost, c->stream));
+    EH_CHECK(hipMemcpyAsync(c->pinned_seq, c->seq, sizeof(SeqDev) * B, hipMemcpyDeviceToHost, c->stream));
+    EH_CHECK(hipStreamSynchronize(c->stream));
+    for (int s = 0; s < B; s++) kn[s] = c->pinned_seq[s].kn_old;
+    return 0;
+}
+
+}
diff --git a/rebvo_amd/edgehip.py b/rebvo_amd/edgehip.py
--- a/rebvo_amd/edgehip.py
+++ b/rebvo_amd/edgehip.py
@@ -258,7 +258,7 @@
     "edgehip_create", "edgehip_destroy", "edgehip_last_error", "edgehip_abi_version", "edgehip_sync",
     "edgehip_stream", "edgehip_box_widths", "edgehip_upload_rgb", "edgehip_upload_rgb_device",
     "edgehip_stage_a", "edgehip_get_kn", "edgehip_quantile", "edgehip_build_field", "edgehip_try_velrot",
-    "edgehip_download_resid", "edgehip_minimizer_rv", "edgehip_forward_match", "edgehip_rotate_keylines",
+    "edgehip_download_resid", "edgehip_minimizer_rv", "edgehip_read_keep_counts", "edgehip_forward_match", "edgehip_rotate_keylines",
     "edgehip_directed_matching", "edgehip_regularize_ekf", "edgehip_rescale", "edgehip_process_frame",
     "edgehip_next_slot", "edgehip_cur_slot", "edgehip_read_nav", "edgehip_reset", "edgehip_get_state",
     "edgehip_set_state", "edgehip_get_framecount", "edgehip_set_framecount", "edgehip_download_keylines", "edgehip_download_keylines_batch",
@@ -604,6 +604,11 @@
     def minimizer_rv(self, slot_new, slot_old):
         self._ck(self.lib.edgehip_minimizer_rv(self.ctx, slot_new, slot_old))
 
+    def read_keep_counts(self):
+        nk, kn = np.zeros(self.nseq, np.int32), np.zeros(self.nseq, np.int32)
+        self._ck(self.lib.edgehip_read_keep_counts(self.ctx, nk.ctypes.data_as(C.c_void_p), kn.ctypes.data_as(C.c_void_p)))
+        return nk, kn
+
     def forward_match(self, slot_old, slot_new):
         self._ck(self.lib.edgehip_forward_match(self.ctx, slot_old, slot_new))
 
```

Result: no change. 133,400, median of 2 (+0.5%).
